# nghorbani/moshpp

Hardware: AMD Instinct MI355X
Metric: solved mocap frames/sec (Stage-II) (higher is better)
Workload: dtype f64

## Files before the change

### moshpp_amd/csrc/chain_solve.hip

```cpp
#include "moshii_dev.h"
#include <utility>
#include <type_traits>
#if defined(__HIP_DEVICE_COMPILE__)
#define MOSHII_OPAQUE(x) __asm__ __volatile__("" : "+v"(x))
#else
#define MOSHII_OPAQUE(x) do {} while (0)
#endif
__device__ __forceinline__ double uni64(double v) {
#if defined(__HIP_DEVICE_COMPILE__)
    return __hiloint2double(__builtin_amdgcn_readfirstlane(__double2hiint(v)), __builtin_amdgcn_readfirstlane(__double2loint(v)));
#else
    return v;
#endif
}

namespace moshii {

typedef double v2d __attribute__((vector_size(16)));

#ifdef MOSHII_PROFILE
__device__ long long g_prof[64];
#define MOSHII_TRACE_N 8192
__device__ long long g_trace[8][MOSHII_TRACE_N][4];
#define TRACE_STAMP(co, seq, ev) do { if (threadIdx.x == 0 && blockIdx.x < 8u * (co).G && (blockIdx.x & 7u) == 0u && (seq) < MOSHII_TRACE_N) g_trace[(co).rank][(seq)][(ev)] = wall_clock64(); } while (0)
#define PROF_BEGIN() long long _pt = clock64()
#define PROF_LAP(slot) do { __syncthreads(); if (threadIdx.x == 0 && blockIdx.x == 0) { long long _n = clock64(); g_prof[slot] += _n - _pt; _pt = _n; } else { _pt = 0; } } while (0)
#define PROF_COUNT(slot) do { if (threadIdx.x == 0 && blockIdx.x == 0) g_prof[slot] += 1; } while (0)
#define PROF_MARK() do { if (threadIdx.x == 0 && blockIdx.x == 0) g_prof[63] = clock64(); } while (0)
#define PROF_LAP_EXT(slot) do { __syncthreads(); if (threadIdx.x == 0 && blockIdx.x == 0) { long long _n = clock64(); g_prof[slot] += _n - g_prof[63]; g_prof[63] = _n; } } while (0)
#define PROF_T(var) const long long var = clock64()
#define PROF_ACC(slot, var) do { if (threadIdx.x == 0 && blockIdx.x == 0) g_prof[slot] += clock64() - var; } while (0)
#else
#define PROF_BEGIN() do {} while (0)
#define PROF_LAP(slot) do {} while (0)
#define PROF_COUNT(slot) do {} while (0)
#define PROF_MARK() do {} while (0)
#define PROF_LAP_EXT(slot) do {} while (0)
#define PROF_T(var) do {} while (0)
#define PROF_ACC(slot, var) do {} while (0)
#define TRACE_STAMP(co, seq, ev) do {} while (0)
#endif

enum { S_KBEST = 0, S_PRIOR_SS = 1, S_FAIL = 2, S_TMP0 = 3, S_TMP1 = 4, S_TMP2 = 5, S_TMP3 = 6, S_PRIOR_REF = 7, S_PRIOR_KB0 = 8, S_BATON = 9, S_ABORT = 10,
       S_V0 = 11, S_V1 = 12,
       S_COOP_SEQ = 13, S_COOP_FAIL = 14
     };

struct Ctx {
    double *pose, *trans, *pose_t, *trans_t, *pose_prev, *vtarget, *fullpose;
    double *feat, *B, *omega, *Rw, *tw, *Rloc, *acol, *Jl;
    double *vposed, *vpos, *msim, *res, *vconst, *vshp, *shp0;
    double *xb, *ell, *score, *px0, *ps0;
    double *g, *dsd, *dgn, *ddl, *y;
    double *red, *scal;
    unsigned long long* anc;
    int *visidx, *colpid, *colprior, *pid2prior, *jointslot, *kfree, *colq, *ksum, *kconst;
    double *big, *Jh, *Jrow, *Lm, *Trot, *xjs, *rest;
    int* tjs;
};

struct FrameParams {
    const double* obs;
    double wt_data, wt_pose, wt_poseH, wt_velo;
    int has_velo, use_fingers, nobs;
    double wt_poseF;
    int use_face, use_shape, has_stay;
    int v0, v1;
};

struct Sse { double data, prior, velo, hand, total, face, shape, stay; };

template <int CTRL>
__device__ __forceinline__ double dpp_f64(double v) {
    const int lo = __builtin_amdgcn_update_dpp(0, __double2loint(v), CTRL, 0xf, 0xf, false);
    const int hi = __builtin_amdgcn_update_dpp(0, __double2hiint(v), CTRL, 0xf, 0xf, false);
    return __hiloint2double(hi, lo);
}
__device__ __forceinline__ double readlane_f64(double v, int lane ) {
    const int lo = __builtin_amdgcn_readlane(__double2loint(v), lane);
    const int hi = __builtin_amdgcn_readlane(__double2hiint(v), lane);
    return __hiloint2double(hi, lo);
}
enum { DPP_QUAD_1032 = 0xB1, DPP_QUAD_2301 = 0x4E, DPP_ROW_HALF_MIRROR = 0x141, DPP_ROW_MIRROR = 0x140 };
#if defined(__HIP_DEVICE_COMPILE__)
template <int K> __device__ __forceinline__ double rowbcast_f64(double v) {
    double r;
    asm volatile("s_nop 1\n\tv_mov_b64_dpp %0, %1 row_newbcast:%2 row_mask:0xf bank_mask:0xf" : "=v"(r) : "v"(v), "n"(K));
    return r;
}
template <int K, bool SETTLE = false> __device__ __forceinline__ void fmac_rowbcast(double& acc, double m, double a) {
    if constexpr (SETTLE) asm volatile("s_nop 1\n\tv_fmac_f64_dpp %0, -%1, %2 row_newbcast:%3 row_mask:0xf bank_mask:0xf" : "+v"(acc) : "v"(m), "v"(a), "n"(K));
    else asm volatile("v_fmac_f64_dpp %0, -%1, %2 row_newbcast:%3 row_mask:0xf bank_mask:0xf" : "+v"(acc) : "v"(m), "v"(a), "n"(K));
}
#else
template <int K> __device__ __forceinline__ double rowbcast_f64(double v) { return __shfl(v, K, 16); }
template <int K, bool SETTLE = false> __device__ __forceinline__ void fmac_rowbcast(double& acc, double m, double a) { acc = fma(-__shfl(m, K, 16), a, acc); }
#endif

__device__ __forceinline__ double wave_sum(double v) {
    v += dpp_f64<DPP_QUAD_1032>(v);
    v += dpp_f64<DPP_QUAD_2301>(v);
    v += dpp_f64<DPP_ROW_HALF_MIRROR>(v);
    v += dpp_f64<DPP_ROW_MIRROR>(v);
    return (readlane_f64(v, 0) + readlane_f64(v, 16)) + (readlane_f64(v, 32) + readlane_f64(v, 48));
}
__device__ __forceinline__ void wave_sum3(double& a, double& b, double& c) {
    a += dpp_f64<DPP_QUAD_1032>(a); b += dpp_f64<DPP_QUAD_1032>(b); c += dpp_f64<DPP_QUAD_1032>(c);
    a += dpp_f64<DPP_QUAD_2301>(a); b += dpp_f64<DPP_QUAD_2301>(b); c += dpp_f64<DPP_QUAD_2301>(c);
    a += dpp_f64<DPP_ROW_HALF_MIRROR>(a); b += dpp_f64<DPP_ROW_HALF_MIRROR>(b); c += dpp_f64<DPP_ROW_HALF_MIRROR>(c);
    a += dpp_f64<DPP_ROW_MIRROR>(a); b += dpp_f64<DPP_ROW_MIRROR>(b); c += dpp_f64<DPP_ROW_MIRROR>(c);
    a = (readlane_f64(a, 0) + readlane_f64(a, 16)) + (readlane_f64(a, 32) + readlane_f64(a, 48));
    b = (readlane_f64(b, 0) + readlane_f64(b, 16)) + (readlane_f64(b, 32) + readlane_f64(b, 48));
    c = (readlane_f64(c, 0) + readlane_f64(c, 16)) + (readlane_f64(c, 32) + readlane_f64(c, 48));
}
__device__ __forceinline__ double wave_max(double v) {
    v = fmax(v, dpp_f64<DPP_QUAD_1032>(v));
    v = fmax(v, dpp_f64<DPP_QUAD_2301>(v));
    v = fmax(v, dpp_f64<DPP_ROW_HALF_MIRROR>(v));
    v = fmax(v, dpp_f64<DPP_ROW_MIRROR>(v));
    return fmax(fmax(readlane_f64(v, 0), readlane_f64(v, 16)), fmax(readlane_f64(v, 32), readlane_f64(v, 48)));
}

__device__ __forceinline__ void block_sum3(double& a, double& b, double& c, double* red) {
    wave_sum3(a, b, c);
    __syncthreads();
    const int tid = threadIdx.x;
    if ((tid & 63) == 0) { red[(tid >> 6) * 3 + 0] = a; red[(tid >> 6) * 3 + 1] = b; red[(tid >> 6) * 3 + 2] = c; }
    __syncthreads();
    a = (red[0] + red[3]) + (red[6] + red[9]);
    b = (red[1] + red[4]) + (red[7] + red[10]);
    c = (red[2] + red[5]) + (red[8] + red[11]);
}
__device__ __forceinline__ void block_sum4(double& a, double& b, double& c, double& d, double* red) {
    wave_sum3(a, b, c);
    d = wave_sum(d);
    __syncthreads();
    const int tid = threadIdx.x;
    if ((tid & 63) == 0) { red[(tid >> 6) * 4 + 0] = a; red[(tid >> 6) * 4 + 1] = b; red[(tid >> 6) * 4 + 2] = c; red[(tid >> 6) * 4 + 3] = d; }
    __syncthreads();
    a = (red[0] + red[4]) + (red[8] + red[12]);
    b = (red[1] + red[5]) + (red[9] + red[13]);
    c = (red[2] + red[6]) + (red[10] + red[14]);
    d = (red[3] + red[7]) + (red[11] + red[15]);
}
__device__ __forceinline__ void block_max_sum3(double& mx, double& a, double& b, double& c, double* red) {
    wave_sum3(a, b, c);
    mx = wave_max(mx);
    __syncthreads();
    const int tid = threadIdx.x;
    if ((tid & 63) == 0) { red[(tid >> 6) * 4 + 0] = a; red[(tid >> 6) * 4 + 1] = b; red[(tid >> 6) * 4 + 2] = c; red[(tid >> 6) * 4 + 3] = mx; }
    __syncthreads();
    a = (red[0] + red[4]) + (red[8] + red[12]);
    b = (red[1] + red[5]) + (red[9] + red[13]);
    c = (red[2] + red[6]) + (red[10] + red[14]);
    mx = fmax(fmax(red[3], red[7]), fmax(red[11], red[15]));
}
__device__ __forceinline__ double block_sum(double a, double* red) {
    double b = 0.0, c = 0.0;
    block_sum3(a, b, c, red);
    return a;
}
__device__ __forceinline__ double block_max(double a, double* red) {
    a = wave_max(a);
    __syncthreads();
    const int tid = threadIdx.x;
    if ((tid & 63) == 0) red[tid >> 6] = a;
    __syncthreads();
    return fmax(fmax(red[0], red[1]), fmax(red[2], red[3]));
}

#if defined(__HIP_DEVICE_COMPILE__)
#define MOSHII_DRAIN_VMEM() asm volatile("s_waitcnt vmcnt(0)" ::: "memory")
#else
#define MOSHII_DRAIN_VMEM() do {} while (0)
#endif
__device__ __forceinline__ unsigned long long f64_bits(double v) { unsigned long long b; __builtin_memcpy(&b, &v, 8); return b; }
__device__ __forceinline__ double bits_f64(unsigned long long b) { double v; __builtin_memcpy(&v, &b, 8); return v; }
__device__ __forceinline__ void coop_st(MOSHII_GP(unsigned long long) p, double v) {
    __hip_atomic_store(p, f64_bits(v), __ATOMIC_RELAXED, __HIP_MEMORY_SCOPE_AGENT);
}
__device__ __forceinline__ double coop_ld(MOSHII_GP(unsigned long long) p) {
    return bits_f64(__hip_atomic_load(p, __ATOMIC_RELAXED, __HIP_MEMORY_SCOPE_AGENT));
}
#if defined(__HIP_DEVICE_COMPILE__)
__device__ __forceinline__ void coop_st_l2(MOSHII_GP(unsigned long long) p, unsigned long long v) {
    asm volatile("global_store_dwordx2 %0, %1, off sc0" :: "v"(p), "v"(v) : "memory");
}
__device__ __forceinline__ unsigned long long coop_ld_l2(MOSHII_GP(unsigned long long) p) {
    unsigned long long v;
    asm volatile("global_load_dwordx2 %0, %1, off sc0 nt\n\ts_waitcnt vmcnt(0)" : "=v"(v) : "v"(p) : "memory");
    return v;
}
__device__ __forceinline__ void coop_st32_l2(MOSHII_GP(unsigned int) p, unsigned v) {
    asm volatile("global_store_dword %0, %1, off sc0" :: "v"(p), "v"(v) : "memory");
}
__device__ __forceinline__ unsigned coop_ld32_l2(MOSHII_GP(unsigned int) p) {
    unsigned v;
    asm volatile("global_load_dword %0, %1, off sc0 nt\n\ts_waitcnt vmcnt(0)" : "=v"(v) : "v"(p) : "memory");
    return v;
}
#endif
template <bool L2> __device__ __forceinline__ void coop_st64(MOSHII_GP(unsigned long long) p, unsigned long long v) {
#if defined(__HIP_DEVICE_COMPILE__)
    if constexpr (L2) { coop_st_l2(p, v); return; }
#endif
    __hip_atomic_store(p, v, __ATOMIC_RELAXED, __HIP_MEMORY_SCOPE_AGENT);
}
template <bool L2> __device__ __forceinline__ unsigned long long coop_ld64(MOSHII_GP(unsigned long long) p) {
#if defined(__HIP_DEVICE_COMPILE__)
    if constexpr (L2) return coop_ld_l2(p);
#endif
    return __hip_atomic_load(p, __ATOMIC_RELAXED, __HIP_MEMORY_SCOPE_AGENT);
}
template <bool L2> __device__ __forceinline__ void coop_st32(MOSHII_GP(unsigned int) p, unsigned v) {
#if defined(__HIP_DEVICE_COMPILE__)
    if constexpr (L2) { coop_st32_l2(p, v); return; }
#endif
    __hip_atomic_store(p, v, __ATOMIC_RELAXED, __HIP_MEMORY_SCOPE_AGENT);
}
template <bool L2> __device__ __forceinline__ unsigned coop_ld32(MOSHII_GP(unsigned int) p) {
#if defined(__HIP_DEVICE_COMPILE__)
    if constexpr (L2) return coop_ld32_l2(p);
#endif
    return __hip_atomic_load(p, __ATOMIC_RELAXED, __HIP_MEMORY_SCOPE_AGENT);
}
__device__ __forceinline__ unsigned coop_begin(const Ctx& cx) { return (unsigned)__builtin_amdgcn_readfirstlane((int)cx.scal[S_COOP_SEQ]) + 1u; }
__device__ __forceinline__ MOSHII_GP(unsigned long long) coop_slot(const CoopCtx& co, unsigned seq, int r) {
    return co.slots + ((size_t)(seq & 1u) * co.G + r) * co.slot_doubles;
}
#if defined(__HIP_DEVICE_COMPILE__) && !defined(MOSHII_COOP_NO_BUF)
typedef unsigned coop_u4 __attribute__((ext_vector_type(4)));
struct CoopSlot { __amdgpu_buffer_rsrc_t rs; };
__device__ __forceinline__ CoopSlot coop_slot16(const CoopCtx& co, unsigned seq, int r) {
    CoopSlot cs;
    cs.rs = __builtin_amdgcn_make_buffer_rsrc((void*)coop_slot(co, seq, r), 0, co.slot_doubles * 8, 0x00020000);
    return cs;
}
template <bool L2 = false>
__device__ __forceinline__ void coop_st16(const CoopSlot& cs, int off16, double a, double b) {
    const unsigned long long ba = f64_bits(a), bb = f64_bits(b);
    const coop_u4 v = {(unsigned)ba, (unsigned)(ba >> 32), (unsigned)bb, (unsigned)(bb >> 32)};
    if constexpr (L2) __builtin_amdgcn_raw_buffer_store_b128(v, cs.rs, off16 * 16, 0, 1);
    else __builtin_amdgcn_raw_buffer_store_b128(v, cs.rs, off16 * 16, 0, 16);
}
template <bool L2 = false>
__device__ __forceinline__ void coop_ld16(const CoopSlot& cs, int off16, double& a, double& b) {
    coop_u4 v;
    if constexpr (L2) v = __builtin_amdgcn_raw_buffer_load_b128(cs.rs, off16 * 16, 0, 3);
    else v = __builtin_amdgcn_raw_buffer_load_b128(cs.rs, off16 * 16, 0, 16);
    a = bits_f64(((unsigned long long)v[1] << 32) | v[0]);
    b = bits_f64(((unsigned long long)v[3] << 32) | v[2]);
}
#else
struct CoopSlot { MOSHII_GP(unsigned long long) p; };
__device__ __forceinline__ CoopSlot coop_slot16(const CoopCtx& co, unsigned seq, int r) { CoopSlot cs; cs.p = coop_slot(co, seq, r); return cs; }
template <bool L2 = false>
__device__ __forceinline__ void coop_st16(const CoopSlot& cs, int off16, double a, double b) { coop_st(cs.p + 2 * (size_t)off16, a); coop_st(cs.p + 2 * (size_t)off16 + 1, b); }
template <bool L2 = false>
__device__ __forceinline__ void coop_ld16(const CoopSlot& cs, int off16, double& a, double& b) { a = coop_ld(cs.p + 2 * (size_t)off16); b = coop_ld(cs.p + 2 * (size_t)off16 + 1); }
#endif
__device__ __forceinline__ void coop_skew(const CoopCtx& co, unsigned seq) {
    if (co.skew != 0) {
        unsigned h = (seq * 2654435761u) ^ ((unsigned)co.rank * 40503u + (unsigned)co.skew * 977u);
        h ^= h >> 13; h *= 0x5bd1e995u; h ^= h >> 15;
        for (unsigned i = h & 3u; i > 0u; --i) __builtin_amdgcn_s_sleep(127);
    }
}
template <bool L2 = false>
__device__ __forceinline__ bool coop_publish_wait(const CoopCtx& co, const Ctx& cx, unsigned seq) {
    const int tid = threadIdx.x;
    coop_skew(co, seq);
    PROF_T(_tp0);
    MOSHII_DRAIN_VMEM();
    __syncthreads();
    PROF_ACC(33, _tp0);
    PROF_T(_tp1);
#if defined(MOSHII_COOP_FENCES)
    if (tid == 0) __hip_atomic_store(co.flags + co.rank, seq, __ATOMIC_RELEASE, __HIP_MEMORY_SCOPE_AGENT);
#else
    if (tid == 0) coop_st32<L2>(co.flags + co.rank, seq);
#endif
    TRACE_STAMP(co, seq, 1);
    if (tid < co.G && cx.scal[S_COOP_FAIL] == 0.0) {
        bool ok = true;
        unsigned spins = 0;
        while ((int)(coop_ld32<L2>(co.flags + tid) - seq) < 0) {
            __builtin_amdgcn_s_sleep(1);
            if ((++spins & 255u) == 0u)
                if (spins > (1u << 21) || __hip_atomic_load(co.flags + co.G, __ATOMIC_RELAXED, __HIP_MEMORY_SCOPE_AGENT) != 0u) { ok = false; break; }
        }
        if (!ok) {
            __hip_atomic_store(co.flags + co.G, 1u, __ATOMIC_RELAXED, __HIP_MEMORY_SCOPE_AGENT);
            cx.scal[S_COOP_FAIL] = 1.0;
        }
    }
    __syncthreads();
#if defined(MOSHII_COOP_FENCES)
    __builtin_amdgcn_fence(__ATOMIC_ACQUIRE, "agent");
#endif
    PROF_ACC(34, _tp1);
    TRACE_STAMP(co, seq, 2);
    return cx.scal[S_COOP_FAIL] == 0.0;
}
__device__ __forceinline__ void coop_end(const Ctx& cx, unsigned seq) {
    __syncthreads();
    if (threadIdx.x == 0) cx.scal[S_COOP_SEQ] = (double)seq;
    __syncthreads();
}
template <int NS, bool L2>
__device__ __forceinline__ bool coop_exchange_small_(const CoopCtx& co, const Ctx& cx, unsigned seq, const double (&mine)[NS], double* land) {
    const int tid = threadIdx.x;
    const int goff = co.slot_doubles - 32;
    coop_skew(co, seq);
    if (tid < 2 * NS) {
        double v = mine[0];
#pragma unroll
        for (int k = 1; k < NS; ++k) if ((tid >> 1) == k) v = mine[k];
        const unsigned long long b = f64_bits(v);
        const unsigned half = (tid & 1) ? (unsigned)(b >> 32) : (unsigned)b;
        coop_st64<L2>(coop_slot(co, seq, co.rank) + goff + tid, ((unsigned long long)seq << 32) | half);
    }
    TRACE_STAMP(co, seq, 1);
    if (tid < co.G * 2 * NS && cx.scal[S_COOP_FAIL] == 0.0) {
        const int r = tid / (2 * NS), k = tid - r * 2 * NS;
        auto* g = coop_slot(co, seq, r) + goff + k;
        unsigned long long x;
        unsigned spins = 0;
        bool ok = true;
        while (((x = coop_ld64<L2>(g)) >> 32) != seq) {
            __builtin_amdgcn_s_sleep(1);
            if ((++spins & 255u) == 0u)
                if (spins > (1u << 21) || __hip_atomic_load(co.flags + co.G, __ATOMIC_RELAXED, __HIP_MEMORY_SCOPE_AGENT) != 0u) { ok = false; break; }
        }
        if (!ok) {
            __hip_atomic_store(co.flags + co.G, 1u, __ATOMIC_RELAXED, __HIP_MEMORY_SCOPE_AGENT);
            cx.scal[S_COOP_FAIL] = 1.0;
        }
        reinterpret_cast<unsigned*>(land)[tid] = (unsigned)x;
    }
    __syncthreads();
    TRACE_STAMP(co, seq, 2);
    return cx.scal[S_COOP_FAIL] == 0.0;
}
template <int NS>
__device__ __forceinline__ bool coop_exchange_small(const CoopCtx& co, const Ctx& cx, unsigned seq, const double (&mine)[NS], double* land) {
    return coop_exchange_small_<NS, false>(co, cx, seq, mine, land);
}

__device__ __forceinline__ void rodrigues_dev(const double* r, double* R, double* Jl) {
    const double x = r[0], y = r[1], z = r[2];
    const double t2 = x * x + y * y + z * z;
    double a, b, c;
    if (t2 < 1e-6) {
        a = 1.0 - t2 / 6.0 + t2 * t2 / 120.0;
        b = 0.5 - t2 / 24.0 + t2 * t2 / 720.0;
        c = 1.0 / 6.0 - t2 / 120.0 + t2 * t2 / 5040.0;
    } else {
        const double t = sqrt(t2);
        double s, co;
        sincos(t, &s, &co);
        a = s / t;
        b = (1.0 - co) / t2;
        c = (t - s) / (t2 * t);
    }
    const double K2[9] = {x * x - t2, x * y, x * z, x * y, y * y - t2, y * z, x * z, y * z, z * z - t2};
    const double Km[9] = {0.0, -z, y, z, 0.0, -x, -y, x, 0.0};
#pragma unroll
    for (int e = 0; e < 9; ++e) {
        const double id = (e == 0 || e == 4 || e == 8) ? 1.0 : 0.0;
        R[e] = id + a * Km[e] + b * K2[e];
        Jl[e] = id + b * Km[e] + c * K2[e];
    }
}

__device__ __forceinline__ void rodrigues_R(const double* r, double* R) {
    const double x = r[0], y = r[1], z = r[2];
    const double t2 = x * x + y * y + z * z;
    double a, b;
    if (t2 < 1e-6) {
        a = 1.0 - t2 / 6.0 + t2 * t2 / 120.0;
        b = 0.5 - t2 / 24.0 + t2 * t2 / 720.0;
    } else {
        const double t = sqrt(t2);
        double s, co;
        sincos(t, &s, &co);
        a = s / t;
        b = (1.0 - co) / t2;
    }
    const double K2[9] = {x * x - t2, x * y, x * z, x * y, y * y - t2, y * z, x * z, y * z, z * z - t2};
    const double Km[9] = {0.0, -z, y, z, 0.0, -x, -y, x, 0.0};
#pragma unroll
    for (int e = 0; e < 9; ++e) R[e] = ((e == 0 || e == 4 || e == 8) ? 1.0 : 0.0) + a * Km[e] + b * K2[e];
}

__device__ __forceinline__ void mat3_mul(const double* A, const double* Bm, double* C) {
#pragma unroll
    for (int i = 0; i < 3; ++i)
#pragma unroll
        for (int j = 0; j < 3; ++j)
            C[i * 3 + j] = A[i * 3 + 0] * Bm[0 * 3 + j] + A[i * 3 + 1] * Bm[1 * 3 + j] + A[i * 3 + 2] * Bm[2 * 3 + j];
}
__device__ __forceinline__ void mat3_vec(const double* A, double x, double y, double z, double& ox, double& oy, double& oz) {
    ox = A[0] * x + A[1] * y + A[2] * z;
    oy = A[3] * x + A[4] * y + A[5] * z;
    oz = A[6] * x + A[7] * y + A[8] * z;
}

__device__ __forceinline__ void marker_eval(const double* c, const double* v0, const double* v1, const double* v2,
                                            double* mk, double* L ) {
    const double e1[3] = {v1[0] - v0[0], v1[1] - v0[1], v1[2] - v0[2]};
    const double e2[3] = {v2[0] - v0[0], v2[1] - v0[1], v2[2] - v0[2]};
    const double l1 = sqrt(e1[0] * e1[0] + e1[1] * e1[1] + e1[2] * e1[2]);
    const double f1[3] = {e1[0] / l1, e1[1] / l1, e1[2] / l1};
    const double nv[3] = {e1[1] * e2[2] - e1[2] * e2[1], e1[2] * e2[0] - e1[0] * e2[2], e1[0] * e2[1] - e1[1] * e2[0]};
    const double ln = sqrt(nv[0] * nv[0] + nv[1] * nv[1] + nv[2] * nv[2]);
    const double f2[3] = {nv[0] / ln, nv[1] / ln, nv[2] / ln};
    const double f3[3] = {f1[1] * f2[2] - f1[2] * f2[1], f1[2] * f2[0] - f1[0] * f2[2], f1[0] * f2[1] - f1[1] * f2[0]};
#pragma unroll
    for (int i = 0; i < 3; ++i) mk[i] = v0[i] + c[0] * f1[i] + c[1] * f2[i] + c[2] * f3[i];
    if (L == nullptr) return;
    double D1[9], D2[9];
#pragma unroll
    for (int i = 0; i < 3; ++i)
#pragma unroll
        for (int j = 0; j < 3; ++j) {
            const double id = (i == j) ? 1.0 : 0.0;
            D1[i * 3 + j] = (id - f1[i] * f1[j]) / l1;
            D2[i * 3 + j] = (id - f2[i] * f2[j]) / ln;
        }
    const double N1[9] = {0.0, e2[2], -e2[1], -e2[2], 0.0, e2[0], e2[1], -e2[0], 0.0};
    const double N2[9] = {0.0, -e1[2], e1[1], e1[2], 0.0, -e1[0], -e1[1], e1[0], 0.0};
    double F21[9], F22[9];
    mat3_mul(D2, N1, F21);
    mat3_mul(D2, N2, F22);
    const double S1[9] = {0.0, -f1[2], f1[1], f1[2], 0.0, -f1[0], -f1[1], f1[0], 0.0};
    const double S2[9] = {0.0, -f2[2], f2[1], f2[2], 0.0, -f2[0], -f2[1], f2[0], 0.0};
    double T1[9], T2[9], T3[9];
    mat3_mul(S2, D1, T1);
    mat3_mul(S1, F21, T2);
    mat3_mul(S1, F22, T3);
#pragma unroll
    for (int i = 0; i < 3; ++i)
#pragma unroll
        for (int j = 0; j < 3; ++j) {
            const int e = i * 3 + j;
            const double de1 = c[0] * D1[e] + c[1] * F21[e] + c[2] * (T2[e] - T1[e]);
            const double de2 = c[1] * F22[e] + c[2] * T3[e];
            const double id = (i == j) ? 1.0 : 0.0;
            L[i * 9 + j] = id - de1 - de2;
            L[i * 9 + 3 + j] = de1;
            L[i * 9 + 6 + j] = de2;
        }
}

__device__ __forceinline__ double fullpose_entry(const ModelDev& md, const double* pose, int d) {
    const int bd = md.body_dof, nhf = md.nhand_full;
    if (d < bd) return pose[d];
    const int h = d - bd;
    const int lo = md.col_lo[h], hi = md.col_hi[h];
    double v0 = md.hands_mean[h], v1 = 0.0;
    int i = lo;
    for (; i + 2 <= hi; i += 2) {
        v0 += pose[bd + i] * md.comps[i * nhf + h];
        v1 += pose[bd + i + 1] * md.comps[(i + 1) * nhf + h];
    }
    if (i < hi) v0 += pose[bd + i] * md.comps[i * nhf + h];
    return v0 + v1;
}

__device__ __forceinline__ void posedirs_partial(const Ctx& cx, const AttachDev& at, const int* klist, int nk,
                                                 const double* base, double* dst) {
    const int tid = threadIdx.x;
    const int Nv = at.Nv, Nvp = at.Nvp, Nvh = Nvp >> 1;
    for (int it = tid; it < 3 * Nvh; it += MOSHII_TPB) {
        const int i = it / Nvh, a2 = it - i * Nvh;
        double s0x = 0.0, s0y = 0.0, s1x = 0.0, s1y = 0.0, s2x = 0.0, s2y = 0.0;
        const auto* pp = gptr(reinterpret_cast<const v2d*>(at.Pt)) + (size_t)(i * 9) * Nvh + a2;
        constexpr int PB = 3;
        for (int idx0 = 0; idx0 < nk; idx0 += PB) {
            v2d q[PB][9];
            int kk[PB];
#pragma unroll
            for (int u = 0; u < PB; ++u) {
                kk[u] = klist[min(idx0 + u, nk - 1)];
                const auto* pk = pp + (size_t)((kk[u] - 1) * 27) * Nvh;
#pragma unroll
                for (int e = 0; e < 9; ++e) q[u][e] = pk[(size_t)e * Nvh];
            }
#pragma unroll
            for (int u = 0; u < PB; ++u) {
                if (idx0 + u < nk) {
                    const double* f = &cx.feat[kk[u] * 9];
#pragma unroll
                    for (int e = 0; e < 9; e += 3) {
                        s0x += q[u][e][0] * f[e]; s0y += q[u][e][1] * f[e];
                        s1x += q[u][e + 1][0] * f[e + 1]; s1y += q[u][e + 1][1] * f[e + 1];
                        s2x += q[u][e + 2][0] * f[e + 2]; s2y += q[u][e + 2][1] * f[e + 2];
                    }
// ... 1616 lines not shown
                                    for (int i = 0; i < 4; ++i) acc.c[t][i] += own[4 * t + i];
                                }
                        } else if (wanted(r0 + u)) {
#pragma unroll
                            for (int t = 0; t < NT; ++t)
                                if (4 * t + wv < NE) {
#pragma unroll
                                    for (int i = 0; i < 4; ++i) acc.c[t][i] += v[u][4 * t + i];
                                }
                        }
                    }
                }
                if (has_prior) {
                    if (NUP + RB * NUA > 48) {
#pragma unroll
                        for (int u = 0; u < NUP; ++u) coop_ld16<L2>(sp, (NUA + u) * MOSHII_TPB + tid, pv[2 * u], pv[2 * u + 1]);
                    }
#pragma unroll
                    for (int e = 0; e < NE; ++e) pblk[e] = pv[e];
                    gqp = pv[NE];
                }
                }
            }
        };
        exchange(std::false_type());
        if (tid < n) cx.dgn[tid] = gqp;
        TRACE_STAMP(co, seq, 3);
        coop_end(cx, seq);
        PROF_LAP(32);
    }
    A.take(acc, cx.big);
    {
        const int ty = tid >> 4, tx = tid & 15, bn = n >> 4;
        if (ty == (n & 15)) {
#pragma unroll
            for (int bi = 0; bi < NBLK; ++bi)
#pragma unroll
                for (int bj = 0; bj <= bi; ++bj)
                    if (bi == bn && bj * 16 + tx < n) cx.g[bj * 16 + tx] = -A.a[bi * (bi + 1) / 2 + bj];
        }
        __syncthreads();
    }
    double* dvec = cx.y;
    const int kb = (np_ > 0) ? (int)cx.scal[S_KBEST] : 0;
    for (int q = tid; q < n; q += MOSHII_TPB) {
        double dg = 0.0, gq = 0.0;
        if (XT && q >= ncp) {
            const int e = q - ncp;
            const double sv_ = pose[md.NP + e];
            const double w2 = op.wt_shape * op.wt_shape;
            dg += w2; gq -= w2 * sv_;
            if (fp.has_stay) { const double y2 = op.wt_shape_stay * op.wt_shape_stay; dg += y2; gq -= y2 * (sv_ - cx.shp0[e]); }
        } else if (q >= 3) {
            const int pid = cx.colpid[q];
            if (fp.has_velo) { const double w2 = fp.wt_velo * fp.wt_velo; dg += w2; gq -= w2 * (pose[pid] - cx.vtarget[pid]); }
            const int pb = cx.colprior[q];
            if (COOP) { gq += cx.dgn[q]; }
            else if (pb >= 0) {
                const auto* Hk = pr.halfprec + (size_t)kb * np_ * np_ + pb;
                const auto* mu = pr.means + (size_t)kb * np_;
                double s0 = 0.0, s1 = 0.0;
                for (int b0 = 0; b0 < np_; b0 += 32) {
                    double h[32];
#pragma unroll
                    for (int k = 0; k < 32; ++k) h[k] = Hk[(size_t)min(b0 + k, np_ - 1) * np_];
#pragma unroll
                    for (int k = 0; k < 32; k += 2) {
                        const int b = b0 + k;
                        s0 = fma(h[k] * ((b < np_) ? 1.0 : 0.0), cx.xb[min(b, np_ - 1)] - mu[min(b, np_ - 1)], s0);
                        s1 = fma(h[k + 1] * ((b + 1 < np_) ? 1.0 : 0.0), cx.xb[min(b + 1, np_ - 1)] - mu[min(b + 1, np_ - 1)], s1);
                    }
                }
                gq -= fp.wt_pose * fp.wt_pose * (s0 + s1);
            }
            if (fp.use_fingers) {
                if (op.nfinger > 0 && pid >= op.finger[0] && pid <= op.finger[op.nfinger - 1]) {
                    const double w2 = fp.wt_poseH * fp.wt_poseH; dg += w2; gq -= w2 * pose[pid];
                }
            }
            if constexpr (XT) {
                if (fp.use_face && op.nface > 0 && pid >= op.face[0] && pid <= op.face[op.nface - 1]) {
                    const double w2 = fp.wt_poseF * fp.wt_poseF; dg += w2; gq -= w2 * pose[pid];
                }
            }
            if (op.njangle > 0)
                for (int i = 0; i < op.njangle; ++i)
                    if (op.jangle[i] == pid) {
                        const double e = exp(pose[pid]);
                        const double r = (e * e) * (fp.wt_pose * op.wt_jangle), d = 2.0 * r;
                        dg += d * d; gq -= d * r;
                    }
        }
        dvec[q] = dg;
        cx.g[q] += gq;
    }
    __syncthreads();
    A.add_diag(dvec, n);
    if constexpr (COOP) {
#pragma unroll
        for (int e = 0; e < AReg<NBLK>::NE; ++e) A.a[e] += pblk[e];
    } else {
        if (np_ > 0) A.add_prior(fp.wt_pose * fp.wt_pose, pr.halfprec + (size_t)kb * np_ * np_, np_, cx.colprior, n);
    }
    __syncthreads();
    PROF_LAP(8);
}

__device__ __forceinline__ Ctx make_ctx(double* lds, const ChainLayout& ly) {
    Ctx cx;
    cx.pose = lds + ly.o_pose; cx.trans = lds + ly.o_trans; cx.pose_t = lds + ly.o_pose_t; cx.trans_t = lds + ly.o_trans_t;
    cx.pose_prev = lds + ly.o_pose_prev; cx.vtarget = lds + ly.o_vtarget; cx.fullpose = lds + ly.o_fullpose;
    cx.Jl = lds + ly.o_Jl; cx.feat = lds + ly.o_feat; cx.B = lds + ly.o_B; cx.omega = lds + ly.o_omega; cx.Rw = lds + ly.o_Rw; cx.tw = lds + ly.o_tw;
    cx.Rloc = lds + ly.o_Rloc; cx.acol = lds + ly.o_acol;
    cx.vshp = lds + ly.o_vshp; cx.shp0 = lds + ly.o_shp0;
    cx.vconst = lds + ly.o_vconst; cx.vposed = lds + ly.o_vposed; cx.vpos = lds + ly.o_vpos; cx.msim = lds + ly.o_msim; cx.res = lds + ly.o_res;
    cx.xb = lds + ly.o_xb; cx.ell = lds + ly.o_ell; cx.score = lds + ly.o_score; cx.px0 = lds + ly.o_px0; cx.ps0 = lds + ly.o_ps0;
    cx.g = lds + ly.o_g; cx.dsd = lds + ly.o_dsd; cx.dgn = lds + ly.o_dgn; cx.ddl = lds + ly.o_ddl; cx.y = lds + ly.o_y;
    cx.red = lds + ly.o_red; cx.scal = lds + ly.o_scal;
    cx.anc = reinterpret_cast<unsigned long long*>(lds + ly.o_anc);
    int* ints = reinterpret_cast<int*>(lds + ly.o_ints);
    cx.visidx = ints + ly.i_visidx; cx.colpid = ints + ly.i_colpid; cx.colprior = ints + ly.i_colprior;
    cx.pid2prior = ints + ly.i_pid2prior; cx.jointslot = ints + ly.i_jointslot; cx.kfree = ints + ly.i_kfree;
    cx.colq = ints + ly.i_colq; cx.ksum = ints + ly.i_ksum; cx.kconst = ints + ly.i_kconst;
    cx.big = lds + ly.o_big;
    cx.Jh = cx.big + ly.t_Jh; cx.Jrow = cx.big + ly.t_Jrow; cx.Lm = cx.big + ly.t_Lm; cx.Trot = cx.big + ly.t_Trot;
    cx.xjs = cx.big + ly.t_xjs; cx.rest = cx.big + ly.t_rest;
    cx.tjs = reinterpret_cast<int*>(cx.big + ly.t_tjs);

    return cx;
}

template <class T>
__device__ __forceinline__ T uniform_load(const T* p) {
    static_assert(sizeof(T) % 4 == 0, "word-sized descriptors only");
    T out;
    int* o = reinterpret_cast<int*>(&out);
    const int* q = reinterpret_cast<const int*>(p);
#pragma unroll
    for (int i = 0; i < (int)(sizeof(T) / 4); ++i) o[i] = __builtin_amdgcn_readfirstlane(q[i]);
    return out;
}

struct KArgsMirror { const ChainDev* chains; ModelDev md; PriorDev pr; OptsDev op; ChainLayout ly; int n_chains; };
#if defined(__HIP_DEVICE_COMPILE__) && !defined(MOSHII_NO_KARGS)
typedef const KArgsMirror __attribute__((address_space(4)))* KArgsPtr;
__device__ __forceinline__ KArgsPtr kargs_of(const KernelCtx* kc) {
    const unsigned long long v = kc->kargs;
    return (KArgsPtr)(((unsigned long long)(unsigned)__builtin_amdgcn_readfirstlane((int)(v >> 32)) << 32) | (unsigned)__builtin_amdgcn_readfirstlane((int)v));
}
#define MOSHII_CTX_FROM_KARGS(kc) const KArgsPtr ka_ = kargs_of(kc); const ChainLayout ly = ka_->ly; const ModelDev md = ka_->md; const PriorDev pr = ka_->pr; const OptsDev op = ka_->op;
#else
#define MOSHII_CTX_FROM_KARGS(kc) const ChainLayout ly = uniform_load(&(kc)->ly); const ModelDev md = uniform_load(&(kc)->md); const PriorDev pr = uniform_load(&(kc)->pr); const OptsDev op = uniform_load(&(kc)->op);
#endif

template <int NBLK>
__device__ __noinline__ bool coop_rs_reduce(unsigned seq_) {
    extern __shared__ __attribute__((aligned(16))) double lds[];
    const KernelCtx* kc = reinterpret_cast<const KernelCtx*>(lds);
    const ChainLayout ly = uniform_load(&kc->ly);
    const Ctx cx = make_ctx(lds, ly);
    const CoopCtx co = uniform_load(&kc->co);
    constexpr int NT = JtJAcc<NBLK>::NT, NE = AReg<NBLK>::NE;
    const int tid = threadIdx.x;
    const int wv = __builtin_amdgcn_readfirstlane(tid >> 6);
    unsigned seq = (unsigned)__builtin_amdgcn_readfirstlane((int)seq_);
    const int TPR = (NT + co.G - 1) / co.G, tlo = co.rank * TPR, thi = min(NT, tlo + TPR);
    v4d sums[NT];
#pragma unroll
    for (int t = 0; t < NT; ++t)
        if (t >= tlo && t < thi && 4 * t + wv < NE) {
            double v[MOSHII_COOP_MAXG][4];
#pragma unroll
            for (int r = 0; r < MOSHII_COOP_MAXG; ++r)
                if (r < co.G) {
                    const CoopSlot sr = coop_slot16(co, seq, r);
                    coop_ld16(sr, (2 * t) * MOSHII_TPB + tid, v[r][0], v[r][1]);
                    coop_ld16(sr, (2 * t + 1) * MOSHII_TPB + tid, v[r][2], v[r][3]);
                }
            v4d sum = v4d{0.0, 0.0, 0.0, 0.0};
#pragma unroll
            for (int r = 0; r < MOSHII_COOP_MAXG; ++r)
                if (r < co.G) {
#pragma unroll
                    for (int i = 0; i < 4; ++i) sum[i] += v[r][i];
                }
            sums[t] = sum;
        }
    coop_end(cx, seq);
    seq = coop_begin(cx);
    const CoopSlot mine2 = coop_slot16(co, seq, co.rank);
#pragma unroll
    for (int t = 0; t < NT; ++t)
        if (t >= tlo && t < thi && 4 * t + wv < NE) {
            coop_st16(mine2, (2 * t) * MOSHII_TPB + tid, sums[t][0], sums[t][1]);
            coop_st16(mine2, (2 * t + 1) * MOSHII_TPB + tid, sums[t][2], sums[t][3]);
        }
    return coop_publish_wait(co, cx, seq);
}

template <bool XT, bool COOP>
__device__ __noinline__ Sse eval_forward_fn(const uint8_t* visrow, int o_pose, int o_trans, int i_klist, int nk,
                                            int o_vbase, int light) {
    extern __shared__ __attribute__((aligned(16))) double lds[];
    const KernelCtx* kc = reinterpret_cast<const KernelCtx*>(lds);
    MOSHII_CTX_FROM_KARGS(kc)
    const AttachDev at = uniform_load(&kc->at);
    const FrameParams fp = uniform_load(reinterpret_cast<const FrameParams*>(kc->fp_raw));
    const Ctx cx = make_ctx(lds, ly);
    const int* ints = reinterpret_cast<const int*>(lds + ly.o_ints);
    CoopCtx co = CoopCtx();
    if constexpr (COOP) co = uniform_load(&kc->co);
    return eval_forward<XT, COOP>(cx, md, at, pr, op, lds + __builtin_amdgcn_readfirstlane(o_pose), lds + __builtin_amdgcn_readfirstlane(o_trans),
                                  fp, visrow, ints + __builtin_amdgcn_readfirstlane(i_klist), __builtin_amdgcn_readfirstlane(nk),
                                  lds + __builtin_amdgcn_readfirstlane(o_vbase), __builtin_amdgcn_readfirstlane(light) != 0, co);
}

#ifdef MOSHII_ASM_INLINE
#define MOSHII_ASM_LINKAGE __forceinline__
#else
#define MOSHII_ASM_LINKAGE __noinline__
#endif
template <int NBLK, bool XT, bool COOP>
__device__ MOSHII_ASM_LINKAGE typename APass<NBLK, MOSHII_ASM_RET_VEC(NBLK)>::type assemble_fn(int o_pose, int n, int ncp, int nkf, int nfree_hand, double* qs) {
    extern __shared__ __attribute__((aligned(16))) double lds[];
    const KernelCtx* kc = reinterpret_cast<const KernelCtx*>(lds);
    MOSHII_CTX_FROM_KARGS(kc)
    const AttachDev at = uniform_load(&kc->at);
    const FrameParams fp = uniform_load(reinterpret_cast<const FrameParams*>(kc->fp_raw));
    const Ctx cx = make_ctx(lds, ly);
    AReg<NBLK> A;
    CoopCtx co = CoopCtx();
    if constexpr (COOP) co = uniform_load(&kc->co);
    assemble<NBLK, XT, COOP>(cx, ly, md, at, pr, op, lds + __builtin_amdgcn_readfirstlane(o_pose), fp, __builtin_amdgcn_readfirstlane(n),
                             __builtin_amdgcn_readfirstlane(ncp), __builtin_amdgcn_readfirstlane(nkf), __builtin_amdgcn_readfirstlane(nfree_hand), qs, A, co);
    return APass<NBLK, MOSHII_ASM_RET_VEC(NBLK)>::pack(A);
}

__device__ __noinline__ void rigid_init_serial(const Ctx& cx, const FrameParams& fp, const uint8_t* visrow, int M) {
    double am[3] = {0, 0, 0}, bm[3] = {0, 0, 0};
    int cnt = 0;
    for (int m = 0; m < M; ++m) if (visrow[m]) {
        for (int i = 0; i < 3; ++i) { am[i] += cx.msim[m * 3 + i]; bm[i] += fp.obs[m * 3 + i]; }
        ++cnt;
    }
    for (int i = 0; i < 3; ++i) { am[i] /= cnt; bm[i] /= cnt; }
    double G[9] = {0, 0, 0, 0, 0, 0, 0, 0, 0};
    for (int m = 0; m < M; ++m) if (visrow[m])
        for (int i = 0; i < 3; ++i) for (int j = 0; j < 3; ++j)
            G[i * 3 + j] += (cx.msim[m * 3 + i] - am[i]) * (fp.obs[m * 3 + j] - bm[j]);
    double V[9] = {1, 0, 0, 0, 1, 0, 0, 0, 1};
    for (int sweep = 0; sweep < 60; ++sweep) {
        double off = 0.0;
        for (int p = 0; p < 2; ++p) for (int q = p + 1; q < 3; ++q) {
            double al = 0, be = 0, ga = 0;
            for (int i = 0; i < 3; ++i) { al += G[i * 3 + p] * G[i * 3 + p]; be += G[i * 3 + q] * G[i * 3 + q]; ga += G[i * 3 + p] * G[i * 3 + q]; }
            if (fabs(ga) <= 1e-300 || fabs(ga) <= 1e-17 * sqrt(al * be)) continue;
            off = fmax(off, fabs(ga) / sqrt(al * be));
            const double zeta = (be - al) / (2.0 * ga);
            const double t = ((zeta >= 0) ? 1.0 : -1.0) / (fabs(zeta) + sqrt(1.0 + zeta * zeta));
            const double c = 1.0 / sqrt(1.0 + t * t), s = c * t;
            for (int i = 0; i < 3; ++i) {
                const double gp = G[i * 3 + p], gq = G[i * 3 + q];
                G[i * 3 + p] = c * gp - s * gq; G[i * 3 + q] = s * gp + c * gq;
                const double vp = V[i * 3 + p], vq = V[i * 3 + q];
                V[i * 3 + p] = c * vp - s * vq; V[i * 3 + q] = s * vp + c * vq;
            }
        }
        if (off < 1e-15) break;
    }
    double sv[3], U[9];
    int imin = 0, imax = 0;
    for (int c = 0; c < 3; ++c) {
        sv[c] = sqrt(G[0 * 3 + c] * G[0 * 3 + c] + G[1 * 3 + c] * G[1 * 3 + c] + G[2 * 3 + c] * G[2 * 3 + c]);
        if (sv[c] < sv[imin]) imin = c;
        if (sv[c] > sv[imax]) imax = c;
    }
    for (int c = 0; c < 3; ++c) for (int i = 0; i < 3; ++i) U[i * 3 + c] = (sv[c] > 0) ? G[i * 3 + c] / sv[c] : 0.0;
    if (sv[imin] <= 1e-13 * sv[imax]) {
        const int c1 = (imin + 1) % 3, c2 = (imin + 2) % 3;
        U[0 * 3 + imin] = U[1 * 3 + c1] * U[2 * 3 + c2] - U[2 * 3 + c1] * U[1 * 3 + c2];
        U[1 * 3 + imin] = U[2 * 3 + c1] * U[0 * 3 + c2] - U[0 * 3 + c1] * U[2 * 3 + c2];
        U[2 * 3 + imin] = U[0 * 3 + c1] * U[1 * 3 + c2] - U[1 * 3 + c1] * U[0 * 3 + c2];
    }
    double R[9];
    for (int i = 0; i < 3; ++i) for (int j = 0; j < 3; ++j)
        R[i * 3 + j] = V[i * 3 + 0] * U[j * 3 + 0] + V[i * 3 + 1] * U[j * 3 + 1] + V[i * 3 + 2] * U[j * 3 + 2];
    const double det = R[0] * (R[4] * R[8] - R[5] * R[7]) - R[1] * (R[3] * R[8] - R[5] * R[6]) + R[2] * (R[3] * R[7] - R[4] * R[6]);
    if (det < 0.0)
        for (int i = 0; i < 3; ++i) for (int j = 0; j < 3; ++j) R[i * 3 + j] -= 2.0 * V[i * 3 + imin] * U[j * 3 + imin];
    double rx = R[7] - R[5], ry = R[2] - R[6], rz = R[3] - R[1];
    const double s = sqrt((rx * rx + ry * ry + rz * rz) * 0.25);
    double c = (R[0] + R[4] + R[8] - 1.0) * 0.5;
    c = fmin(1.0, fmax(-1.0, c));
    const double theta = acos(c);
    double rv[3];
    if (s < 1e-5) {
        if (c > 0) { rv[0] = rv[1] = rv[2] = 0.0; }
        else {
            double x = sqrt(fmax((R[0] + 1.0) * 0.5, 0.0));
            double y = sqrt(fmax((R[4] + 1.0) * 0.5, 0.0)) * ((R[1] >= 0) ? 1.0 : -1.0);
            double z = sqrt(fmax((R[8] + 1.0) * 0.5, 0.0)) * ((R[2] >= 0) ? 1.0 : -1.0);
            if (fabs(x) < fabs(y) && fabs(x) < fabs(z) && ((R[5] > 0) != (y * z > 0))) z = -z;
            const double nn = sqrt(x * x + y * y + z * z);
            rv[0] = x * theta / nn; rv[1] = y * theta / nn; rv[2] = z * theta / nn;
        }
    } else {
        const double k = 0.5 * theta / s;
        rv[0] = rx * k; rv[1] = ry * k; rv[2] = rz * k;
    }
    cx.pose[0] = rv[0]; cx.pose[1] = rv[1]; cx.pose[2] = rv[2];
    for (int i = 0; i < 3; ++i) cx.trans[i] = bm[i] - (R[i * 3 + 0] * am[0] + R[i * 3 + 1] * am[1] + R[i * 3 + 2] * am[2]);
}

template <int NBLK, bool XT, bool COOP>
__device__ Sse run_phase(const Ctx& cx, const ChainLayout& ly, const ModelDev& md, const AttachDev& at, const PriorDev& pr,
                         const OptsDev& op, const FrameParams& fp, const uint8_t* visrow, MOSHII_GP(const int) ids, int nids, int nshp,
                         double* qs, double e3,
                         bool rigid, bool eval_only, bool reuse, Sse& carried, bool& at_pose, int& fwd_set, int set_id, int& vc_key,
                         int& tab_key, int& n_iter, int& n_fev, int& fail, const CoopCtx& co) {
    const int tid = threadIdx.x;
    const int ncp = 3 + nids;
    const int n = ncp + (XT ? nshp : 0);
    const int NPX = XT ? ly.NPX : md.NP;
    if (!eval_only && tab_key != set_id) {
        tab_key = set_id;
        for (int i = tid; i < md.NP; i += MOSHII_TPB) cx.colq[i] = -1;
        __syncthreads();
        for (int q = tid; q < n; q += MOSHII_TPB) {
            const int pid = (q < 3) ? -1 : ((q < ncp) ? ids[q - 3] : md.NP + (q - ncp));
            cx.colpid[q] = pid;
            cx.colprior[q] = (pid >= 0 && pid < md.NP) ? cx.pid2prior[pid] : -1;
            if (pid >= 0 && pid < md.NP) cx.colq[pid] = q;
        }
        if (tid == 0) {
            for (int k = 0; k < md.K; ++k) cx.jointslot[k] = -1;
            for (int i = 0; i < nids; ++i) {
                const int pid = ids[i];
                if (pid < md.body_dof) cx.jointslot[pid / 3] = 0;
                else for (int k = md.body_dof / 3; k < md.K; ++k) cx.jointslot[k] = 0;
            }
            int c = 0;
            for (int k = 0; k < md.K; ++k) if (cx.jointslot[k] == 0) { cx.jointslot[k] = c; cx.kfree[c] = k; ++c; }
            cx.scal[S_TMP0] = (double)c;
            int nh = 0;
            for (int i = 0; i < nids; ++i) nh += (ids[i] >= md.body_dof) ? 1 : 0;
            cx.scal[S_TMP2] = (double)nh;
            int ns = 0, nc = 0;
            for (int k = 1; k < md.K; ++k) { if (cx.jointslot[k] >= 0) cx.ksum[ns++] = k; else cx.kconst[nc++] = k; }
            cx.scal[S_TMP3] = (double)ns;
        }
        __syncthreads();
    }
    const int nkf = (int)cx.scal[S_TMP0], nfree_hand = (int)cx.scal[S_TMP2];
    const int nks = (int)cx.scal[S_TMP3];
    const int nkc = md.K - 1 - nks;
    if (vc_key != set_id) {
        for (int d = tid; d < md.P; d += MOSHII_TPB) cx.fullpose[d] = fullpose_entry(md, cx.pose, d);
        __syncthreads();
        if (tid < md.K) {
            double R[9];
            rodrigues_R(&cx.fullpose[3 * tid], R);
#pragma unroll
            for (int e = 0; e < 9; ++e) cx.feat[tid * 9 + e] = R[e] - ((e == 0 || e == 4 || e == 8) ? 1.0 : 0.0);
        }
        __syncthreads();
        if constexpr (COOP) posedirs_partial_range(cx, at, cx.kconst, nkc, at.vsh, cx.vconst, 3 * co.mlo, 3 * co.mhi);
        else posedirs_partial(cx, at, cx.kconst, nkc, at.vsh, cx.vconst);
        __syncthreads();
        vc_key = set_id;
    }
    AReg<NBLK> A;
    A.zero();
    if (tid == 0) {
        extern __shared__ __attribute__((aligned(16))) double lds[];
        static_assert(sizeof(FrameParams) <= sizeof(KernelCtx::fp_raw), "KernelCtx::fp_raw too small");
        *reinterpret_cast<FrameParams*>(reinterpret_cast<KernelCtx*>(lds)->fp_raw) = fp;
    }
    for (int i = tid; i < NPX; i += MOSHII_TPB) cx.pose_t[i] = cx.pose[i];
    if (tid < 3) cx.trans_t[tid] = cx.trans[tid];
    __syncthreads();
    Sse last;
    double sse = 0.0, delta = op.delta0, norm_sd = 0.0, norm_gn = 0.0, step = 0.0, p2 = 0.0, gd = 0.0;
    double dAd = 0.0, dl_dd = 0.0, dl_gs = 0.0, dl_ds = 0.0;
    bool init = true, done = false, have_gn = false;
    int iteration = 0;
    bool skip_eval = reuse && !rigid;
    int light = (!rigid && at_pose && fwd_set == set_id) ? 1 : 0;
    while (true) {
        int tid = threadIdx.x; MOSHII_OPAQUE(tid);
        if (skip_eval) { last = carried; skip_eval = false; }
        else { PROF_T(_te); last = eval_forward_fn<XT, COOP>(visrow, ly.o_pose_t, ly.o_trans_t, ly.i_ksum, nks, ly.o_vconst, light); PROF_ACC(15, _te); }
        if constexpr (COOP) { if (cx.scal[S_COOP_FAIL] != 0.0) break; }
        if (!(last.total == last.total)) { fail = 1; break; }
        light = 0;
        at_pose = true;
        fwd_set = set_id;
        if (rigid) {
            if constexpr (COOP) {
                const unsigned seq = coop_begin(cx);
                auto gather = [&](auto l2) {
                    constexpr bool L2 = decltype(l2)::value;
                    auto* mine = coop_slot(co, seq, co.rank);
                    for (int i = 3 * co.mlo + tid; i < 3 * co.mhi; i += MOSHII_TPB) coop_st64<L2>(mine + i, f64_bits(cx.msim[i]));
                    if (tid == 0) coop_st64<L2>(mine + 3 * at.M, f64_bits((double)co.mlo));
                    if (coop_publish_wait<L2>(co, cx, seq)) {
                        const int M3 = 3 * at.M;
                        for (int i = tid; i < M3; i += MOSHII_TPB) {
                            int r = 0;
                            for (int q = 1; q < co.G; ++q) r += (i >= 3 * (int)bits_f64(coop_ld64<L2>(coop_slot(co, seq, q) + 3 * at.M))) ? 1 : 0;
                            if (r != co.rank) cx.msim[i] = bits_f64(coop_ld64<L2>(coop_slot(co, seq, r) + i));
                        }
                    }
                };
                gather(std::false_type());
                coop_end(cx, seq);
            }
            if (tid == 0) rigid_init_serial(cx, fp, visrow, at.M);
            __syncthreads();
            for (int i = tid; i < NPX; i += MOSHII_TPB) cx.pose_t[i] = cx.pose[i];
            if (tid < 3) cx.trans_t[tid] = cx.trans[tid];
            __syncthreads();
            rigid = false;
            continue;
        }
        if (eval_only) break;
        ++n_fev;
        PROF_T(_t1);
        bool improved = false, do_assemble = false;
        double rho = 0.0;
        if (init) {
            sse = uni64(last.total);
            do_assemble = true;
        } else {
            rho = sse - last.total;
            if (rho > 0.0) rho = rho / (2.0 * gd - dAd);
            improved = rho > 0.0;
            at_pose = improved;
            if (improved) {
                for (int i = tid; i < NPX; i += MOSHII_TPB) cx.pose[i] = cx.pose_t[i];
                if (tid < 3) cx.trans[tid] = cx.trans_t[tid];
                __syncthreads();
                if (e3 > 0.0 && (sse - last.total) / sse < e3) done = true;
                else { do_assemble = true; sse = uni64(last.total); }
            }
        }
        PROF_ACC(23, _t1);
        double pp = 0.0, gg = 0.0, gAg = 0.0;
        if (do_assemble) {
            { PROF_T(_ta); A = APass<NBLK, MOSHII_ASM_RET_VEC(NBLK)>::unpack(assemble_fn<NBLK, XT, COOP>(ly.o_pose, n, ncp, nkf, nfree_hand, qs)); PROF_ACC(16, _ta); }
            if constexpr (COOP) { if (cx.scal[S_COOP_FAIL] != 0.0) break; }
            PROF_T(_t2);
            double gm = 0.0;
            for (int q = tid; q < n; q += MOSHII_TPB) {
                const double gq = cx.g[q];
                const double pq = (q < 3) ? cx.trans[q] : cx.pose[cx.colpid[q]];
                gm = fmax(gm, fabs(gq)); pp += pq * pq; gg += gq * gq;
            }
            gAg = A.quad_partial(cx.g, n, tid);
            block_max_sum3(gm, pp, gg, gAg, cx.red);
            gm = uni64(gm); pp = uni64(pp); gg = uni64(gg); gAg = uni64(gAg);
            if (gm < 1e-15) done = true;
            PROF_ACC(24, _t2);
        }
        PROF_T(_t3);
        if (!init) {
            const double pnorm2 = (improved && do_assemble) ? pp : p2;
            if (rho > 0.9) delta = fmax(delta, 2.5 * step);
            else if (rho < 0.05) delta *= 0.25;
            delta = uni64(delta);
            if (delta <= 1e-15 * sqrt(pnorm2)) done = true;
        }
        if (init || improved) {
            if (!init && iteration >= op.maxiter) done = true;
            if (done) break;
            ++iteration;
            const double csd = gg / gAg;
            norm_sd = uni64(fabs(csd) * sqrt(gg));
            for (int q = tid; q < n; q += MOSHII_TPB) cx.dsd[q] = csd * cx.g[q];
            have_gn = false;
            __syncthreads();
        } else if (done) {
            break;
        }
        init = false;
        PROF_ACC(25, _t3);
        PROF_T(_t4);
        if (norm_sd >= delta) {
            const double sc = delta / norm_sd;
            for (int q = tid; q < n; q += MOSHII_TPB) cx.ddl[q] = sc * cx.dsd[q];
        } else {
            if (!have_gn) {
                constexpr bool BIG = XT && NBLK > 8;
                bool solved;
                PROF_T(_ts);
                if constexpr (BIG) solved = ldl_big<NBLK>(A, qs + (size_t)6 * md.K * op.nshape, cx.big, cx.g, cx.dgn, cx.y, n);
                else solved = ldl_solve<NBLK>(A, ly.o_big, ly.o_g, ly.o_dgn, ly.o_y, n);
                PROF_ACC(17, _ts);
                PROF_ACC(26, _t4);
                if (!solved) {
                    fail = 1;
                    for (int q = tid; q < n; q += MOSHII_TPB) cx.dgn[q] = cx.dsd[q];
                    __syncthreads();
                }
                double sg = 0.0;
                dl_dd = 0.0; dl_gs = 0.0; dl_ds = 0.0;
                for (int q = tid; q < n; q += MOSHII_TPB) {
                    const double dg_ = cx.dgn[q], dsq = cx.dsd[q], df = dg_ - dsq;
                    sg += dg_ * dg_; dl_dd += df * df; dl_gs += dg_ * dsq; dl_ds += df * dsq;
                }
                block_sum4(sg, dl_dd, dl_gs, dl_ds, cx.red);
                dl_dd = uni64(dl_dd); dl_gs = uni64(dl_gs); dl_ds = uni64(dl_ds);
                norm_gn = uni64(sqrt(sg));
                have_gn = true;
            }
            if (norm_gn <= delta) {
                for (int q = tid; q < n; q += MOSHII_TPB) cx.ddl[q] = cx.dgn[q];
            } else {
                const double delta_sq = delta * delta;
                const double sqnorm_sd = norm_sd * norm_sd;
                const double pnow = dl_dd * delta_sq + dl_gs * dl_gs - (norm_gn * norm_gn) * sqnorm_sd;
                const double beta = (delta_sq - sqnorm_sd) / (dl_ds + sqrt(pnow));
                for (int q = tid; q < n; q += MOSHII_TPB) cx.ddl[q] = cx.dsd[q] + beta * (cx.dgn[q] - cx.dsd[q]);
            }
        }
        __syncthreads();
        PROF_T(_t5);
        double s2 = 0.0;
        p2 = 0.0; gd = 0.0;
        for (int q = tid; q < n; q += MOSHII_TPB) {
            const double dq = cx.ddl[q];
            const double pq = (q < 3) ? cx.trans[q] : cx.pose[cx.colpid[q]];
            s2 += dq * dq; p2 += pq * pq; gd += cx.g[q] * dq;
        }
        dAd = A.quad_partial(cx.ddl, n, tid);
        block_sum4(s2, p2, gd, dAd, cx.red);
        p2 = uni64(p2); gd = uni64(gd); dAd = uni64(dAd);
        step = uni64(sqrt(s2));
        if (step <= 1e-15 * sqrt(p2)) break;
        for (int i = tid; i < NPX; i += MOSHII_TPB) cx.pose_t[i] = cx.pose[i];
        if (tid < 3) cx.trans_t[tid] = cx.trans[tid] + cx.ddl[tid];
        __syncthreads();
        for (int q = 3 + tid; q < n; q += MOSHII_TPB) cx.pose_t[cx.colpid[q]] += cx.ddl[q];
        __syncthreads();
        PROF_ACC(27, _t5);
    }
    n_iter += iteration;
    carried = last;
    return last;
}


template <int NBLK, int MINW, bool XT, bool COOP = false>
__global__ __launch_bounds__(MOSHII_TPB, MINW) void k_chain_solve(const ChainDev* __restrict__ chains, ModelDev md, PriorDev pr,
                                                             OptsDev op, ChainLayout ly, int n_chains) {
    extern __shared__ __attribute__((aligned(16))) double lds[];
    const int tid = threadIdx.x;
    int chain_id = blockIdx.x;
    CoopCtx co = CoopCtx();
    if constexpr (COOP) {
        const int G = chains[0].coop.G;
        const int q = blockIdx.x >> 3;
        chain_id = 8 * (q / G) + (blockIdx.x & 7);
        if (chain_id >= n_chains) return;
        const ChainDev* c0 = chains + chain_id;
        co.G = G; co.rank = q % G; co.prior_rank = c0->coop.prior_rank;
        co.mlo = c0->coop.mlo[co.rank]; co.mhi = c0->coop.mlo[co.rank + 1];
        co.prior_bare = c0->coop.mlo[co.prior_rank + 1] == c0->coop.mlo[co.prior_rank];
        co.slot_doubles = c0->coop.slot_doubles; co.slots = c0->coop.slots; co.flags = c0->coop.flags; co.skew = c0->coop.skew;
    }
    const bool lead = !COOP || co.rank == 0;
    const ChainDev* chp = chains + chain_id;
    const AttachDev at = *chp->att;
    const Ctx cx = make_ctx(lds, ly);
    if (tid == 0) {
        KernelCtx* kc = reinterpret_cast<KernelCtx*>(lds);
        kc->ly = ly; kc->md = md; kc->pr = pr; kc->op = op; kc->at = at;
#if defined(__HIP_DEVICE_COMPILE__)
        kc->kargs = (unsigned long long)__builtin_amdgcn_kernarg_segment_ptr();
#if !defined(MOSHII_NO_KARGS)
        {
            const KArgsPtr kk = (KArgsPtr)__builtin_amdgcn_kernarg_segment_ptr();
            if (kk->chains != chains || kk->n_chains != n_chains || kk->ly.total_doubles != ly.total_doubles || kk->md.V != md.V || kk->op.maxiter != op.maxiter)
                __builtin_trap();
        }
#endif
#endif
        if constexpr (COOP) { kc->co = co; cx.scal[S_COOP_SEQ] = 0.0; cx.scal[S_COOP_FAIL] = 0.0; }
    }

    const int NP = md.NP, M = at.M, F = chp->F, skip = chp->skip;
    bool has_prev, first;
    {
        const double* is = chp->init_state;
        const double* ip = chp->init_pose;
        const double* iv = chp->init_prev;
        const double* it = chp->init_trans;
        for (int i = tid; i < NP; i += MOSHII_TPB) {
            cx.pose[i] = is ? is[i] : (ip ? ip[i] : 0.0);
            cx.pose_prev[i] = is ? is[NP + i] : (iv ? iv[i] : 0.0);
            cx.vtarget[i] = 0.0;
            cx.pid2prior[i] = -1;
        }
        if (tid < 3) cx.trans[tid] = is ? is[2 * NP + tid] : (it ? it[tid] : 0.0);
        if constexpr (XT) {
            const double* ish = chp->init_shape;
            for (int e = tid; e < op.nshape; e += MOSHII_TPB) { cx.pose[NP + e] = is ? is[2 * NP + 5 + e] : (ish ? ish[e] : 0.0); cx.shp0[e] = 0.0; }
        }
        has_prev = is ? (is[2 * NP + 3] != 0.0) : (iv != nullptr);
        first = is ? (is[2 * NP + 4] != 0.0) : (chp->first != 0);
    }
    if (tid == 0) cx.scal[S_PRIOR_REF] = 0.0;
    for (int i = tid; i < 8 * pr.npose + 16; i += MOSHII_TPB) cx.ell[i] = 0.0;
    if (tid < md.K) cx.anc[tid] = md.anc[tid];
    for (int i = tid; i < 3 * md.K; i += MOSHII_TPB) cx.Jl[i] = md.J[i];
    __syncthreads();
    for (int b = tid; b < op.nbody; b += MOSHII_TPB) cx.pid2prior[op.body[b]] = b;
    __syncthreads();
    int vc_key = 0, tab_key = 0;
    int rejoin_run = 0;
    int bi_next = 0;
    bool fuse_on = false;
    bool at_pose = false;
    int fwd_set = 0;
    PROF_BEGIN();
#ifdef MOSHII_PROFILE
    const long long _wall0 = wall_clock64();
#endif

    bool tail_cut = false;
    for (int t = 0; t <= F; ++t) {
        PROF_T(_tf);
        if constexpr (!COOP && !XT) {
            if (chp->tail_done != nullptr && chp->tail_can_cut != 0 && t < F && F - t > chp->tail_left) {
                if (tid == 0) cx.scal[S_ABORT] = (double)__hip_atomic_load(chp->tail_done, __ATOMIC_RELAXED, __HIP_MEMORY_SCOPE_AGENT);
                __syncthreads();
                const bool cut = cx.scal[S_ABORT] >= (double)chp->tail_quota;
                __syncthreads();
                if (cut) {
                    auto spoil = [&](double* so, double flag) {
                        for (int i = tid; i < NP; i += MOSHII_TPB) { so[i] = cx.pose[i]; so[NP + i] = cx.pose_prev[i]; }
                        if (tid < 3) so[2 * NP + tid] = cx.trans[tid];
                        if (tid == 3) so[2 * NP + 3] = flag;
                        if (tid == 4) so[2 * NP + 4] = 0.0;
                    };
                    spoil(chp->entry_state, MOSHII_MARK_ENTRY_SPOILED);
                    spoil(chp->final_state, MOSHII_MARK_FINAL_SPOILED);
                    if (tid == 0 && chp->tail_mark != nullptr) *chp->tail_mark = 0x7fffffff;
                    tail_cut = true;
                    break;
                }
            }
        }
        if constexpr (COOP) {
            if (chp->baton != nullptr || chp->nb > 0 || chp->rejoin_tol > 0.0) {
                bool halt = false;
                if (lead) {
                    const int S = 2 * NP + 5;
                    if (rejoin_run >= 2 && t < F) {
                        if (tid == 0 && chp->frames_done) *chp->frames_done = t;
                        halt = true;
                    }
                    if (!halt && bi_next < chp->nb && t == chp->bnd[bi_next] - chp->bnd_off) {
                        double* s1 = chp->run_final + (size_t)bi_next * S;
                        for (int i = tid; i < NP; i += MOSHII_TPB) { s1[i] = cx.pose[i]; s1[NP + i] = cx.pose_prev[i]; }
                        if (tid < 3) s1[2 * NP + tid] = cx.trans[tid];
                        if (tid == 3) s1[2 * NP + 3] = has_prev ? 1.0 : 0.0;
                        if (tid == 4) s1[2 * NP + 4] = first ? 1.0 : 0.0;
                        if (chp->baton != nullptr) {
                            if (tid == 0) {
                                int* st = chp->baton + 2 * (chp->chunk0 + 1 + bi_next);
                                double go = 1.0;
                                if (__hip_atomic_load(st, __ATOMIC_ACQUIRE, __HIP_MEMORY_SCOPE_AGENT) == 1) {
                                    __hip_atomic_store(st + 1, 1, __ATOMIC_RELEASE, __HIP_MEMORY_SCOPE_AGENT);
                                    int spins = 0;
                                    while (__hip_atomic_load(st, __ATOMIC_ACQUIRE, __HIP_MEMORY_SCOPE_AGENT) != 2) {
                                        __builtin_amdgcn_s_sleep(64);
                                        if (++spins > 20000) { go = 0.0; break; }
                                    }
                                }
                                __builtin_amdgcn_fence(__ATOMIC_ACQUIRE, "agent");
                                cx.scal[S_BATON] = go;
                            }
                            __syncthreads();
                            if (cx.scal[S_BATON] == 0.0) { if (tid == 0 && chp->frames_done) *chp->frames_done = t; halt = true; }
                            __syncthreads();
                        }
                        if (!halt) {
                            double* s2 = chp->run_entry + (size_t)(bi_next + 1) * S;
                            for (int i = tid; i < NP; i += MOSHII_TPB) { s2[i] = cx.pose[i]; s2[NP + i] = cx.pose_prev[i]; }
                            if (tid < 3) s2[2 * NP + tid] = cx.trans[tid];
                            if (tid == 3) s2[2 * NP + 3] = has_prev ? 1.0 : 0.0;
                            if (tid == 4) s2[2 * NP + 4] = first ? 1.0 : 0.0;
                            ++bi_next;
                        }
                    }
                    if (!halt && chp->baton != nullptr && t < F) {
                        if (tid == 0) cx.scal[S_ABORT] = (double)__hip_atomic_load(&chp->baton[2 * chp->chunk0 + 1], __ATOMIC_RELAXED, __HIP_MEMORY_SCOPE_AGENT);
                        __syncthreads();
                        if (cx.scal[S_ABORT] != 0.0) {
                            if (tid == 0) {
                                chp->run_entry[(size_t)bi_next * S + 2 * NP + 3] = MOSHII_MARK_ENTRY_SPOILED;
                                int* mark = chp->abort_at + chp->chunk0 + bi_next;
                                if (*mark < chp->bnd_off + t) *mark = chp->bnd_off + t;
                                if (chp->frames_done) *chp->frames_done = -t - 1;
                            }
                            halt = true;
                        }
                        __syncthreads();
                    }
                }
                const unsigned seq = coop_begin(cx);
                const double mine[1] = {halt ? 1.0 : 0.0};
                const bool okx = coop_exchange_small<1>(co, cx, seq, mine, cx.y);
                const double verdict = okx ? cx.y[0] : 1.0;
                coop_end(cx, seq);
                if (verdict != 0.0) break;
            }
        }
        for (int which = 0; which < 2; ++which) {
            double* so = (which == 0) ? ((t == skip) ? chp->entry_state : nullptr) : ((t == F) ? chp->final_state : nullptr);
            if (so == nullptr || !lead) continue;
            for (int i = tid; i < NP; i += MOSHII_TPB) { so[i] = cx.pose[i]; so[NP + i] = cx.pose_prev[i]; }
            if (tid < 3) so[2 * NP + tid] = cx.trans[tid];
            if (tid == 3) so[2 * NP + 3] = has_prev ? 1.0 : 0.0;
            if (tid == 4) so[2 * NP + 4] = first ? 1.0 : 0.0;
            if constexpr (XT) for (int e = tid; e < op.nshape; e += MOSHII_TPB) so[2 * NP + 5 + e] = cx.pose[NP + e];
        }
        if (!COOP && chp->fuse_flags != nullptr) {
            const int S = 2 * NP + 5 + (XT ? op.nshape : 0);
            if (t == skip && chp->entry_state != nullptr) {
                __syncthreads();
                if (tid == 0) { __threadfence(); __hip_atomic_store(&chp->fuse_flags[3 * chp->fuse_c], 1, __ATOMIC_RELEASE, __HIP_MEMORY_SCOPE_AGENT); }
            }
            if (chp->fuse_F == 0 && t == F) {
                __syncthreads();
                if (tid == 0) {
                    __threadfence();
                    __hip_atomic_store(&chp->fuse_flags[3 * chp->fuse_c + 1], 1, __ATOMIC_RELEASE, __HIP_MEMORY_SCOPE_AGENT);
                    __hip_atomic_store(&chp->fuse_flags[3 * chp->fuse_c + 2], 1, __ATOMIC_RELEASE, __HIP_MEMORY_SCOPE_AGENT);
                }
            }
            if (chp->fuse_F > 0 && t == chp->fuse_F) {
                double* sf = chp->run_final - S;
                for (int i = tid; i < NP; i += MOSHII_TPB) { sf[i] = cx.pose[i]; sf[NP + i] = cx.pose_prev[i]; }
                if (tid < 3) sf[2 * NP + tid] = cx.trans[tid];
                if (tid == 3) sf[2 * NP + 3] = has_prev ? 1.0 : 0.0;
                if (tid == 4) sf[2 * NP + 4] = first ? 1.0 : 0.0;
                if constexpr (XT) for (int e = tid; e < op.nshape; e += MOSHII_TPB) sf[2 * NP + 5 + e] = cx.pose[NP + e];
                __syncthreads();
                if (tid == 0) { __threadfence(); __hip_atomic_store(&chp->fuse_flags[3 * chp->fuse_c + 1], 1, __ATOMIC_RELEASE, __HIP_MEMORY_SCOPE_AGENT); }
                bool carry = false;
                auto state_dev = [&](const double* en) {
                    double dv = 0.0, nn = 0.0;
                    for (int i = tid; i < NP; i += MOSHII_TPB) { dv = fmax(dv, fmax(fabs(cx.pose[i] - en[i]), fabs(cx.pose_prev[i] - en[NP + i]))); nn += en[i] + en[NP + i]; }
                    if (tid < 3) dv = fmax(dv, fabs(cx.trans[tid] - en[2 * NP + tid]));
                    if (tid == 3 && (has_prev ? 1.0 : 0.0) != en[2 * NP + 3]) dv = MOSHII_HANDOFF_MISMATCH;
                    if (tid == 4 && (first ? 1.0 : 0.0) != en[2 * NP + 4]) dv = MOSHII_HANDOFF_MISMATCH;
                    if constexpr (XT) for (int e = tid; e < op.nshape; e += MOSHII_TPB) dv = fmax(dv, fabs(cx.pose[NP + e] - en[2 * NP + 5 + e]));
                    if (!(nn == nn)) dv = MOSHII_HANDOFF_MISMATCH;
                    return block_max(dv, cx.red);
                };
                auto wait_flag = [&](int* fl, int patience) {
                    if (tid == 0) {
                        double go = 1.0;
                        int spins = 0;
                        while (__hip_atomic_load(fl, __ATOMIC_ACQUIRE, __HIP_MEMORY_SCOPE_AGENT) != 1) {
                            __builtin_amdgcn_s_sleep(64);
                            if (++spins > patience) { go = 0.0; break; }
                        }
                        __builtin_amdgcn_fence(__ATOMIC_ACQUIRE, "agent");
                        cx.scal[S_BATON] = go;
                    }
                    __syncthreads();
                    const bool ok_ = cx.scal[S_BATON] != 0.0;
                    __syncthreads();
                    return ok_;
                };
                if (chp->fuse_has_next && wait_flag(chp->fuse_flags + 3 * (chp->fuse_c + 1), 2000)) {
                    const double dv = state_dev(chp->run_entry);
                    carry = !(dv <= chp->fuse_tol);
                    if (carry && dv > 1e-6 && chp->fuse_has_prev && wait_flag(chp->fuse_flags + 3 * (chp->fuse_c - 1) + 1, 150)) {
                        const double* lf = chp->run_final - 2 * S;
                        const double* oe = chp->run_entry - S;
                        double dl = 0.0;
                        for (int i = tid; i < 2 * NP + 3; i += MOSHII_TPB) dl = fmax(dl, fabs(lf[i] - oe[i]));
                        dl = block_max(dl, cx.red);
                        if (!(dl <= 1e-6)) carry = false;
                    }
                }
                if (carry && tid == 0) __hip_atomic_store(&chp->baton[2 * chp->chunk0], 1, __ATOMIC_RELEASE, __HIP_MEMORY_SCOPE_AGENT);
                __syncthreads();
                if (tid == 0) { __threadfence(); __hip_atomic_store(&chp->fuse_flags[3 * chp->fuse_c + 2], 1, __ATOMIC_RELEASE, __HIP_MEMORY_SCOPE_AGENT); }
                if (!carry) { if (tid == 0 && chp->frames_done) *chp->frames_done = t; break; }
                if (tid == 0) {
                    int* fl = chp->fuse_flags + 3 * (chp->fuse_c + 1) + 1;
                    double go = 1.0;
                    int spins = 0;
                    while (__hip_atomic_load(fl, __ATOMIC_ACQUIRE, __HIP_MEMORY_SCOPE_AGENT) != 1 ||
                           __hip_atomic_load(fl + 1, __ATOMIC_ACQUIRE, __HIP_MEMORY_SCOPE_AGENT) != 1) {
                        if (__hip_atomic_load(&chp->baton[2 * chp->chunk0 + 1], __ATOMIC_RELAXED, __HIP_MEMORY_SCOPE_AGENT) != 0) { go = 0.0; break; }
                        __builtin_amdgcn_s_sleep(64);
                        if (++spins > 20000) { go = 0.0; break; }
                    }
                    __builtin_amdgcn_fence(__ATOMIC_ACQUIRE, "agent");
                    if (go != 0.0 && chp->fuse_count != nullptr) atomicAdd(chp->fuse_count, 1);
                    cx.scal[S_BATON] = go;
                }
                __syncthreads();
                if (cx.scal[S_BATON] == 0.0) { if (tid == 0 && chp->frames_done) *chp->frames_done = t; break; }
                double* s2 = chp->run_entry;
                for (int i = tid; i < NP; i += MOSHII_TPB) { s2[i] = cx.pose[i]; s2[NP + i] = cx.pose_prev[i]; }
                if (tid < 3) s2[2 * NP + tid] = cx.trans[tid];
                if (tid == 3) s2[2 * NP + 3] = has_prev ? 1.0 : 0.0;
                if (tid == 4) s2[2 * NP + 4] = first ? 1.0 : 0.0;
                if constexpr (XT) for (int e = tid; e < op.nshape; e += MOSHII_TPB) s2[2 * NP + 5 + e] = cx.pose[NP + e];
                fuse_on = true;
            }
        }
        const bool sweeping = chp->fuse_F == 0 || fuse_on;
        if (!COOP && bi_next < chp->nb && t == chp->bnd[bi_next] - chp->bnd_off) {
            const int S = 2 * NP + 5 + (XT ? op.nshape : 0);
            double* s1 = chp->run_final + (size_t)bi_next * S;
            for (int i = tid; i < NP; i += MOSHII_TPB) { s1[i] = cx.pose[i]; s1[NP + i] = cx.pose_prev[i]; }
            if (tid < 3) s1[2 * NP + tid] = cx.trans[tid];
            if (tid == 3) s1[2 * NP + 3] = has_prev ? 1.0 : 0.0;
            if (tid == 4) s1[2 * NP + 4] = first ? 1.0 : 0.0;
            if constexpr (XT) for (int e = tid; e < op.nshape; e += MOSHII_TPB) s1[2 * NP + 5 + e] = cx.pose[NP + e];
            if (chp->baton != nullptr) {
                if (tid == 0) {
                    int* st = chp->baton + 2 * (chp->chunk0 + 1 + bi_next);
                    double go = 1.0;
                    if (chp->fuse_flags != nullptr) {
                        int* vd = chp->fuse_flags + 3 * (chp->chunk0 + bi_next) + 2;
                        int spins = 0;
                        while (__hip_atomic_load(vd, __ATOMIC_ACQUIRE, __HIP_MEMORY_SCOPE_AGENT) != 1) {
                            __builtin_amdgcn_s_sleep(64);
                            if (++spins > 20000) { go = 0.0; break; }
                        }
                    }
                    if (go != 0.0 && __hip_atomic_load(st, __ATOMIC_ACQUIRE, __HIP_MEMORY_SCOPE_AGENT) == 1) {
                        __hip_atomic_store(st + 1, 1, __ATOMIC_RELEASE, __HIP_MEMORY_SCOPE_AGENT);
                        int spins = 0;
                        while (__hip_atomic_load(st, __ATOMIC_ACQUIRE, __HIP_MEMORY_SCOPE_AGENT) != 2) {
                            __builtin_amdgcn_s_sleep(64);
                            if (++spins > 20000) { go = 0.0; break; }
                        }
                    }
                    if (go != 0.0 && chp->fuse_flags != nullptr) {
                        int* od = chp->fuse_flags + 3 * (chp->chunk0 + 1 + bi_next) + 1;
                        int spins = 0;
                        while (__hip_atomic_load(od, __ATOMIC_ACQUIRE, __HIP_MEMORY_SCOPE_AGENT) != 1) {
                            __builtin_amdgcn_s_sleep(64);
                            if (++spins > 20000) { go = 0.0; break; }
                        }
                    }
                    __builtin_amdgcn_fence(__ATOMIC_ACQUIRE, "agent");
                    cx.scal[S_BATON] = go;
                }
                __syncthreads();
                if (cx.scal[S_BATON] == 0.0) { if (tid == 0 && chp->frames_done) *chp->frames_done = t; break; }
            }
            double* s2 = chp->run_entry + (size_t)(bi_next + 1) * S;
            for (int i = tid; i < NP; i += MOSHII_TPB) { s2[i] = cx.pose[i]; s2[NP + i] = cx.pose_prev[i]; }
            if (tid < 3) s2[2 * NP + tid] = cx.trans[tid];
            if (tid == 3) s2[2 * NP + 3] = has_prev ? 1.0 : 0.0;
            if (tid == 4) s2[2 * NP + 4] = first ? 1.0 : 0.0;
            if constexpr (XT) for (int e = tid; e < op.nshape; e += MOSHII_TPB) s2[2 * NP + 5 + e] = cx.pose[NP + e];
            ++bi_next;
        }
        if (!COOP && chp->baton != nullptr && sweeping && t < F) {
            if (tid == 0) cx.scal[S_ABORT] = (double)__hip_atomic_load(&chp->baton[2 * chp->chunk0 + 1], __ATOMIC_RELAXED, __HIP_MEMORY_SCOPE_AGENT);
            __syncthreads();
            if (cx.scal[S_ABORT] != 0.0) {
                if (tid == 0) {
                    const int S = 2 * NP + 5 + (XT ? op.nshape : 0);
                    chp->run_entry[(size_t)bi_next * S + 2 * NP + 3] = MOSHII_MARK_ENTRY_SPOILED;
                    int* mark = chp->abort_at + chp->chunk0 + bi_next;
                    if (*mark < chp->bnd_off + t) *mark = chp->bnd_off + t;
                    if (chp->frames_done) *chp->frames_done = -t - 1;
                }
                break;
            }
        }
        if (t == F) break;
        const bool record = t >= skip;
        const uint8_t* visrow = chp->vis + (size_t)t * M;
        if (tid < 64) {
            int c = 0, c0 = 0, c1 = 0;
            for (int m0 = 0; m0 < M; m0 += 64) {
                const int m = m0 + tid;
                const bool v = m < M && gptr(visrow)[min(m, M - 1)] != 0;
                const unsigned long long mask = __ballot(v);
                if (v) cx.visidx[c + __popcll(mask & ((1ull << tid) - 1ull))] = m;
                c += __popcll(mask);
                if constexpr (COOP) {
                    c0 += __popcll(__ballot(v && m < co.mlo));
                    c1 += __popcll(__ballot(v && m < co.mhi));
                }
            }
            if (tid == 0) { cx.scal[S_TMP1] = (double)c; cx.scal[S_V0] = (double)c0; cx.scal[S_V1] = (double)c1; }
        }
        __syncthreads();
        const int nobs = (int)cx.scal[S_TMP1];
        if (nobs == 0) {
            int* st = chp->status;
            if (tid == 0 && st && record && lead) st[t] = 1;
            __syncthreads();
            continue;
        }
        FrameParams fp;
        fp.obs = chp->obs + (size_t)t * M * 3;
        fp.nobs = nobs;
        fp.v0 = COOP ? (int)cx.scal[S_V0] : 0;
        fp.v1 = COOP ? (int)cx.scal[S_V1] : nobs;
        const double n_miss = (double)(M - nobs);
        double anneal = 1.0;
        if (n_miss > 0.0) anneal = anneal + (n_miss / (double)M) * op.wt_annealing;
        fp.wt_data = op.wt_data * (op.num_train_markers / (double)nobs);
        const double wt_pose = op.wt_poseB * anneal;
        fp.wt_pose = wt_pose;
        fp.wt_poseH = op.wt_poseH * anneal;
        fp.wt_velo = op.wt_velo;
        fp.use_fingers = 0;
        fp.wt_poseF = 0.0; fp.use_face = 0; fp.use_shape = 0; fp.has_stay = 0;
        if constexpr (XT) {
            fp.wt_poseF = op.wt_poseF * anneal;
            fp.has_stay = (!first && op.wt_shape_stay != 0.0) ? 1 : 0;
            for (int e = tid; e < op.nshape; e += MOSHII_TPB) cx.shp0[e] = cx.pose[NP + e];
        }
        fp.has_velo = has_prev ? 1 : 0;
        if (has_prev)
            for (int i = tid; i < NP; i += MOSHII_TPB) cx.vtarget[i] = cx.pose[i] + (cx.pose[i] - cx.pose_prev[i]);
        if (!first) {
            for (int i = tid; i < NP; i += MOSHII_TPB) cx.pose_prev[i] = cx.pose[i];
            has_prev = true;
        }
        __syncthreads();
        int n_iter = 0, n_fev = 0, fail = 0;
        PROF_ACC(18, _tf);
        Sse fin, carried;
        const bool same_sets = op.same_sets != 0;
        double prev_wt_pose = -1.0;
        int prev_terms = -1;
        for (int kind = first ? 0 : 3; kind < 6; ++kind) {
            const bool round = kind < 3;
            const bool step2 = kind == 4;
            fp.wt_pose = round ? ((kind == 0) ? 10.0 : (kind == 1) ? 5.0 : 1.0) * wt_pose : wt_pose;
            fp.use_fingers = (kind >= 4 && op.nfinger > 0) ? 1 : 0;
            if constexpr (XT) {
                fp.use_face = (kind >= 4 && op.nface > 0) ? 1 : 0;
                fp.use_shape = (kind >= 4 && op.nshape > 0) ? 1 : 0;
            }
            const int terms = fp.use_fingers | (fp.use_face << 1) | (fp.use_shape << 2);
            const bool reuse = at_pose && prev_wt_pose == fp.wt_pose && prev_terms == terms;
            fin = run_phase<NBLK, XT, COOP>(cx, ly, md, at, pr, op, fp, visrow, step2 ? op.step2 : op.step1, step2 ? op.n2 : op.n1,
                                  (XT && step2) ? op.nshape : 0, XT ? chp->qscratch + (COOP ? (size_t)co.rank * chp->coop.qstride : 0) : nullptr,
                                  round ? op.e3_first : op.e3, kind == 0, kind == 5, reuse, carried, at_pose, fwd_set,
                                  (kind >= 4 && !same_sets) ? 2 : 1, vc_key, tab_key, n_iter, n_fev, fail, co);
            prev_wt_pose = fp.wt_pose; prev_terms = terms;
            if constexpr (COOP) { if (cx.scal[S_COOP_FAIL] != 0.0) break; }
        }
        if constexpr (COOP) {
            if (cx.scal[S_COOP_FAIL] != 0.0) break;
        }
        first = false;
        PROF_T(_tr);
        if (lead && record && sweeping && chp->rejoin_tol > 0.0 && chp->pose != nullptr && chp->trans != nullptr) {
            double dv = 0.0;
            const double* po = chp->pose + (size_t)t * NP;
            for (int i = tid; i < NP; i += MOSHII_TPB) dv = fmax(dv, fabs(cx.pose[i] - po[i]));
            if (tid < 3) dv = fmax(dv, fabs(cx.trans[tid] - chp->trans[t * 3 + tid]));
            if constexpr (XT)
                if (chp->shape != nullptr)
                    for (int e = tid; e < op.nshape; e += MOSHII_TPB) dv = fmax(dv, fabs(cx.pose[NP + e] - chp->shape[(size_t)t * op.nshape + e]));
            dv = block_max(dv, cx.red);
            rejoin_run = (dv <= chp->rejoin_tol) ? rejoin_run + 1 : 0;
        }
        if (record) {
            double* o;
            if (lead && (o = chp->pose) != nullptr) for (int i = tid; i < NP; i += MOSHII_TPB) o[(size_t)t * NP + i] = cx.pose[i];
            if (lead && (o = chp->fullpose) != nullptr) for (int i = tid; i < md.P; i += MOSHII_TPB) o[(size_t)t * md.P + i] = cx.fullpose[i];
            if ((o = chp->msim) != nullptr) {
                const int i_lo = COOP ? 3 * co.mlo : 0, i_hi = COOP ? 3 * co.mhi : 3 * M;
                for (int i = i_lo + tid; i < i_hi; i += MOSHII_TPB) o[(size_t)t * 3 * M + i] = cx.msim[i];
            }
            if constexpr (XT)
                if (lead && (o = chp->shape) != nullptr) for (int e = tid; e < op.nshape; e += MOSHII_TPB) o[(size_t)t * op.nshape + e] = cx.pose[NP + e];
            if (tid == 0 && lead) {
                if ((o = chp->trans) != nullptr) { o[t * 3 + 0] = cx.trans[0]; o[t * 3 + 1] = cx.trans[1]; o[t * 3 + 2] = cx.trans[2]; }
                if ((o = chp->errs) != nullptr) {
                    const bool ja = op.njangle > 0;
                    o[t * 8 + 0] = fin.data; o[t * 8 + 1] = fin.prior; o[t * 8 + 2] = fin.velo; o[t * 8 + 3] = ja ? 0.0 : fin.hand;
                    o[t * 8 + 4] = XT ? fin.face : 0.0; o[t * 8 + 5] = XT ? fin.shape : 0.0; o[t * 8 + 6] = XT ? fin.stay : 0.0; o[t * 8 + 7] = ja ? fin.hand : 0.0;
                }
                int* oi;
                if ((oi = chp->iters) != nullptr) { oi[t * 2 + 0] = n_iter; oi[t * 2 + 1] = n_fev; }
                if ((oi = chp->status) != nullptr) oi[t] = fail ? -1 : 0;
            }
        }
        __syncthreads();
        if (lead && rejoin_run > 0 && chp->abort_at != nullptr) {
            const int mark = __hip_atomic_load(chp->abort_at + chp->chunk0 + bi_next, __ATOMIC_RELAXED, __HIP_MEMORY_SCOPE_AGENT);
            if (chp->bnd_off + t < mark) rejoin_run = 0;
        }
        if (!COOP && rejoin_run >= 2 && t + 1 < F) { if (tid == 0 && chp->frames_done) *chp->frames_done = t + 1; break; }
        if (t + 1 == F && tid == 0 && lead && chp->frames_done) *chp->frames_done = F;
        PROF_ACC(19, _tr);
    }
    if constexpr (COOP) {
        if (cx.scal[S_COOP_FAIL] != 0.0 && lead && tid == 0 && chp->run_entry != nullptr) {
            const int S = 2 * NP + 5;
            chp->run_entry[(size_t)bi_next * S + 2 * NP + 3] = MOSHII_MARK_ENTRY_SPOILED;
            if (chp->abort_at != nullptr) chp->abort_at[chp->chunk0 + bi_next] = 0x7fffffff;
        }
        if (chp->baton != nullptr && cx.scal[S_COOP_FAIL] == 0.0) {
            __syncthreads();
            if (tid == 0) __threadfence();
            const unsigned seq = coop_begin(cx);
            const double mine[1] = {0.0};
            coop_exchange_small<1>(co, cx, seq, mine, cx.y);
            coop_end(cx, seq);
        }
    }
    if (lead && chp->baton != nullptr) {
        __syncthreads();
        if (tid == 0) {
            __threadfence();
            __hip_atomic_store(&chp->baton[2 * chp->chunk0], 2, __ATOMIC_RELEASE, __HIP_MEMORY_SCOPE_AGENT);
        }
    }
    if constexpr (!COOP && !XT) {
        if (chp->tail_done != nullptr) {
            (void)tail_cut;
            __syncthreads();
            if (tid == 0) { __threadfence(); atomicAdd(chp->tail_done, 1); }
        }
    }
    PROF_LAP(12);
#ifdef MOSHII_PROFILE
    if (threadIdx.x == 0 && blockIdx.x == 0) g_prof[30] += wall_clock64() - _wall0;
#endif
}

#ifdef MOSHII_DEV_ONLY_NBLK4
template __global__ void k_chain_solve<4, 1, false, false>(const ChainDev*, ModelDev, PriorDev, OptsDev, ChainLayout, int);
template __global__ void k_chain_solve<4, 1, false, true>(const ChainDev*, ModelDev, PriorDev, OptsDev, ChainLayout, int);
#else
#define MOSHII_INSTANTIATE(N, XT_, COOP_) \
    template __global__ void k_chain_solve<N, 1, XT_, COOP_>(const ChainDev*, ModelDev, PriorDev, OptsDev, ChainLayout, int);
MOSHII_INSTANTIATE(2, false, false)
MOSHII_INSTANTIATE(4, false, false)
MOSHII_INSTANTIATE(5, false, false)
MOSHII_INSTANTIATE(7, false, false)
MOSHII_INSTANTIATE(8, false, false)
MOSHII_INSTANTIATE(5, true, false)
MOSHII_INSTANTIATE(8, true, false)
MOSHII_INSTANTIATE(10, true, false)
MOSHII_INSTANTIATE(13, true, false)
MOSHII_INSTANTIATE(4, false, true)
MOSHII_INSTANTIATE(5, false, true)
MOSHII_INSTANTIATE(7, false, true)
MOSHII_INSTANTIATE(8, false, true)
MOSHII_INSTANTIATE(5, true, true)
MOSHII_INSTANTIATE(8, true, true)
MOSHII_INSTANTIATE(10, true, true)
MOSHII_INSTANTIATE(13, true, true)
#undef MOSHII_INSTANTIATE
#endif

__global__ __launch_bounds__(MOSHII_TPB) void k_markers(const AttachDev* __restrict__ attp, ModelDev md, ChainLayout ly,
                                                        const double* __restrict__ pose, const double* __restrict__ trans,
                                                        double* __restrict__ out) {
    extern __shared__ __attribute__((aligned(16))) double lds[];
    const int tid = threadIdx.x;
    const AttachDev at = *attp;
    const Ctx cx = make_ctx(lds, ly);
    const int f = blockIdx.x;
    for (int i = tid; i < md.NP; i += MOSHII_TPB) cx.pose[i] = pose[(size_t)f * md.NP + i];
    if (tid < 3) cx.trans[tid] = trans[(size_t)f * 3 + tid];
    __syncthreads();
    FrameParams fp;
    fp.obs = nullptr; fp.wt_data = 0.0; fp.wt_pose = 0.0; fp.wt_poseH = 0.0; fp.wt_velo = 0.0;
    fp.has_velo = 0; fp.use_fingers = 0; fp.nobs = 0;
    fp.wt_poseF = 0.0; fp.use_face = 0; fp.use_shape = 0; fp.has_stay = 0;
    PriorDev pr; pr.G = 0; pr.npose = 0; pr.means = nullptr; pr.chols = nullptr; pr.halfprec = nullptr; pr.neglogw = nullptr;
    OptsDev op;
    op.nbody = 0; op.nfinger = 0; op.n1 = 0; op.n2 = 0; op.maxiter = 0;
    op.step1 = nullptr; op.step2 = nullptr; op.body = nullptr; op.finger = nullptr;
    op.nface = 0; op.nshape = 0; op.face = nullptr;
    op.njangle = 0; op.wt_jangle = 0.0; op.jangle = nullptr;
    for (int k = 1 + tid; k < md.K; k += MOSHII_TPB) cx.ksum[k - 1] = k;
    for (int i = tid; i < 3 * md.K; i += MOSHII_TPB) cx.Jl[i] = md.J[i];
    __syncthreads();
    fp.v0 = 0; fp.v1 = 0;
    eval_forward<false>(cx, md, at, pr, op, cx.pose, cx.trans, fp, nullptr, cx.ksum, md.K - 1, at.vsh, false);
    for (int i = tid; i < 3 * at.M; i += MOSHII_TPB) out[(size_t)f * 3 * at.M + i] = cx.msim[i];
}

}

extern "C" hipError_t moshii_launch_chain_solve(int nblk, int xt, int n_chains, size_t lds_bytes, hipStream_t stream,
                                                const ChainDev* chains, const ModelDev* md, const PriorDev* pr,
                                                const OptsDev* op, const ChainLayout* ly, int coop_g) {
    using namespace moshii;
    void (*kern)(const ChainDev*, ModelDev, PriorDev, OptsDev, ChainLayout, int) = nullptr;
#ifdef MOSHII_DEV_ONLY_NBLK4
    if (xt || nblk != 4) return hipErrorInvalidValue;
    if (coop_g >= 1) kern = k_chain_solve<4, 1, false, true>; else kern = k_chain_solve<4, 1, false, false>;
// ... 62 lines not shown
```

### moshpp_amd/csrc/moshii_api.hip

```cpp
#include "../../include/moshii.h"
#include "moshii_dev.h"
#include "dev_mem.h"
#include "export_plan.h"
#include "solve_plan.h"
#include "stagei_views.h"

#include <algorithm>
#include <atomic>
#include <cmath>
#include <cstdio>
#include <cstdlib>
#include <cstring>
#include <memory>
#include <mutex>
#include <string>
#include <vector>

extern "C" hipError_t moshii_launch_chain_solve(int nblk, int xt, int n_chains, size_t lds_bytes, hipStream_t stream,
                                                const ChainDev* chains, const ModelDev* md, const PriorDev* pr,
                                                const OptsDev* op, const ChainLayout* ly, int coop_g);
extern "C" hipError_t moshii_launch_markers(int F, size_t lds_bytes, hipStream_t stream, const AttachDev* att,
                                            const ModelDev* md, const ChainLayout* ly, const double* pose,
                                            const double* trans, double* out);
extern "C" hipError_t moshii_launch_lbs_f32(hipStream_t stream, const ModelDev* md, int F, const float* pose,
// ... 1105 lines not shown
        if (g == 0) return 0;
    }
    if (g == 1) return 0;
    if (g < 0 || g > MOSHII_COOP_MAXG) return -2;
    return g;
}

struct SolveDims { int xt, nshape, nmax, nblk, nkfmax, nhj, G, npose; };

int check_opts(moshii_model_t m, moshii_prior_t prior, const moshii_solve_opts* o, SolveDims* d) {
    if (!m->betas_set) return fail(MOSHII_ERR_ARG, "moshii_model_set_betas has not been called");
    if (o->n_body > 0 && (!prior || prior->npose != o->n_body)) return fail(MOSHII_ERR_ARG, "prior npose must equal n_body");
    if (o->n_step1 < 0 || o->n_step2 < 0 || o->n_step1 > m->NP || o->n_step2 > m->NP) return fail(MOSHII_ERR_ARG, "bad free-variable lists");
    const int NP = m->NP;
    const int nshape = o->n_shape;
    if (nshape < 0 || o->n_face < 0) return fail(MOSHII_ERR_ARG, "bad Step-2 extras");
    if (nshape > 0 && nshape != m->nshape) return fail(MOSHII_ERR_ARG, "n_shape must equal the block of moshii_model_set_free_shape");
    if (o->n_face > 0 && !o->face_ids) return fail(MOSHII_ERR_ARG, "face_ids missing");
    for (int i = 1; i < o->n_face; ++i)
        if (o->face_ids[i] != o->face_ids[i - 1] + 1) return fail(MOSHII_ERR_UNSUPPORTED, "face ids must be contiguous");
    if (o->n_jangle < 0 || (o->n_jangle > 0 && !o->jangle_ids)) return fail(MOSHII_ERR_ARG, "bad joint-angle term");
    for (int i = 0; i < o->n_jangle; ++i)
        if (o->jangle_ids[i] < 0 || o->jangle_ids[i] >= NP) return fail(MOSHII_ERR_ARG, "joint-angle id out of range");
    if (o->n_jangle > 0 && o->n_finger > 0)
        return fail(MOSHII_ERR_UNSUPPORTED, "a joint-angle term and finger ids in one solve (no SMAL model has fingers)");
    const int xt = (nshape > 0 || o->n_face > 0) ? 1 : 0;
    const int nmax = 3 + std::max(o->n_step1, o->n_step2 + nshape);
    int nblk = pick_nblk(nmax, xt != 0);
    if (nblk < 0) return fail(MOSHII_ERR_UNSUPPORTED, xt ? "more than 207 unknowns per step" : "more than 124 free pose variables per step");
    if (const char* e = getenv("MOSHII_FORCE_NBLK")) nblk = std::max(nblk, atoi(e));
    auto count_kf = [&](const int32_t* ids, int n) {
        std::vector<char> need(m->K, 0);
        for (int i = 0; i < n; ++i) {
            if (ids[i] < 0 || ids[i] >= NP) return -1;
            if (ids[i] < m->body_dof) need[ids[i] / 3] = 1;
            else for (int k = m->body_dof / 3; k < m->K; ++k) need[k] = 1;
        }
        int c = 0; for (char b : need) c += b; return c;
    };
    const int kf1 = count_kf(o->step1_ids, o->n_step1), kf2 = count_kf(o->step2_ids, o->n_step2);
    if (kf1 < 0 || kf2 < 0) return fail(MOSHII_ERR_ARG, "free pose id out of range");
    if (o->n_finger > 0)
        for (int i = 1; i < o->n_finger; ++i)
            if (o->finger_ids[i] != o->finger_ids[i - 1] + 1) return fail(MOSHII_ERR_UNSUPPORTED, "finger ids must be contiguous");
    bool hand_free = false;
    for (int i = 0; i < o->n_step1; ++i) hand_free |= o->step1_ids[i] >= m->body_dof;
    for (int i = 0; i < o->n_step2; ++i) hand_free |= o->step2_ids[i] >= m->body_dof;
    d->xt = xt; d->nshape = nshape; d->nmax = nmax; d->nblk = nblk;
    d->nkfmax = std::max(1, std::max(kf1, kf2));
    d->nhj = hand_free ? (m->K - m->body_dof / 3) : 0;
    d->G = prior ? prior->G : 0; d->npose = prior ? prior->npose : 0;
    return MOSHII_OK;
}

int choose_layout(moshii_model_t m, const SolveDims& d, int Mmax, int Nvmax, int NWmax, int n_workgroups, int coop_g, LaunchCfg* cfg) {
    const int xt = d.xt, nmax = d.nmax, npose = d.npose;
    int nblk = d.nblk;
    auto layout = [&](int Tm) { return make_layout(m, Mmax, Nvmax, NWmax, npose, d.G, nmax, d.nkfmax, Tm, nblk, d.nhj, d.nshape); };
    const int n_cu = cu_count();
    int budget = 160 * 1024;
    if (const char* e = getenv("MOSHII_LDS_BUDGET")) budget = atoi(e);
    int Tm;
    ChainLayout ly;
    if (coop_g == -1) coop_g = solve_plan::own_group_size(Mmax, d.nkfmax, npose > 0, !xt && nblk < 4);
    if (coop_g > 0 && ((!xt && nmax + 1 > 8 * 16) || (long long)coop_g * std::max(n_workgroups, 1) > n_cu)) coop_g = 0;
    if (coop_g > 0) {
        if (!xt && nblk < 4) nblk = 4;
        if (nmax + 1 > nblk * 16) return fail(MOSHII_ERR_UNSUPPORTED, "cooperative chains: too many unknowns");
        if (coop_g > MOSHII_COOP_MAXG) return fail(MOSHII_ERR_ARG, "cooperative chains: at most 8 workgroups per chain");
        cfg->coop_prior_frac = (npose > 0) ? ((coop_g >= 3) ? (xt ? 0.5 : 0.0) : 0.4) : 1.0;
        if (const char* e = getenv("MOSHII_COOP_PRIOR_FRAC")) cfg->coop_prior_frac = std::min(1.0, std::max(0.0, atof(e)));
        int mlo[MOSHII_COOP_MAXG + 1];
        coop_split(Mmax, coop_g, cfg->coop_prior_frac, mlo);
        int share = 2;
        for (int r = 0; r < coop_g; ++r) share = std::max(share, mlo[r + 1] - mlo[r]);
        Tm = std::min(40, share + 1);
        ly = layout(Tm);
        while (Tm > 2 && (size_t)ly.total_doubles * 8 > (size_t)budget) ly = layout(--Tm);
        cfg->coop = CoopLayout(nblk, Mmax, coop_g);
        cfg->coop_prior_rank = coop_g - 1;
    } else
    if (const char* e = getenv("MOSHII_TM")) {
        Tm = std::max(1, std::min(40, atoi(e)));
        ly = layout(Tm);
    } else {
        int best = -1, best_cost = 0;
        for (int t = std::min(40, std::max(2, Mmax)); t >= 2; --t) {
            const ChainLayout lt = layout(t);
            if ((size_t)lt.total_doubles * 8 > (size_t)budget) continue;
            const int full = Mmax / t, rem = Mmax % t;
            const int rounds = full * ((t * d.nkfmax + 255) / 256) + (rem ? (rem * d.nkfmax + 255) / 256 : 0);
            const int cost = 3 * rounds + 4 * (full + (rem ? 1 : 0));
            if (best < 0 || cost < best_cost) { best = t; best_cost = cost; }
        }
        if (best < 0) best = 2;
        Tm = best;
        ly = layout(Tm);
    }
    const size_t lds_bytes = (size_t)ly.total_doubles * sizeof(double);
    if (lds_bytes > 160 * 1024) return fail(MOSHII_ERR_UNSUPPORTED, "problem does not fit the 160 KiB LDS of a CU");
    cfg->nblk = nblk; cfg->xt = xt; cfg->ly = ly; cfg->lds_bytes = lds_bytes;
    cfg->coop_g = coop_g;
    return MOSHII_OK;
}

int upload_ids(moshii_model_t m, moshii_prior_t prior, const moshii_solve_opts* o, hipStream_t stream, size_t extra_bytes, LaunchCfg* cfg,
               size_t* ctl_off) {
    const int nshape = o->n_shape, njangle = std::max(0, o->n_jangle);
    const size_t nids = (size_t)o->n_step1 + o->n_step2 + o->n_body + o->n_finger + o->n_face + njangle;
    const size_t need = sizeof(int) * (nids + 16) + 64 + extra_bytes;
    int rc = m->scratch.reserve(need, stream);
    if (rc) return rc;
    std::vector<int> ids;
    ids.reserve(nids);
    const size_t e1 = 0, e2 = e1 + o->n_step1, eb = e2 + o->n_step2, ef = eb + o->n_body;
    ids.insert(ids.end(), o->step1_ids, o->step1_ids + o->n_step1);
    ids.insert(ids.end(), o->step2_ids, o->step2_ids + o->n_step2);
    ids.insert(ids.end(), o->body_ids, o->body_ids + o->n_body);
    ids.insert(ids.end(), o->finger_ids, o->finger_ids + o->n_finger);
    const size_t efc = ids.size();
    ids.insert(ids.end(), o->face_ids, o->face_ids + o->n_face);
    const size_t eja = ids.size();
    if (njangle > 0) ids.insert(ids.end(), o->jangle_ids, o->jangle_ids + njangle);
    char* dbase = m->scratch.ptr;
    if (!ids.empty()) {
        HIP_TRY(hipMemcpyAsync(dbase, ids.data(), ids.size() * sizeof(int), hipMemcpyHostToDevice, stream));
        HIP_TRY(hipStreamSynchronize(stream));
    }
    *ctl_off = (ids.size() * sizeof(int) + 63) & ~size_t(63);

    OptsDev& od = cfg->od;
    od.wt_data = o->wt_data; od.wt_velo = o->wt_velo; od.wt_poseB = o->wt_poseB; od.wt_poseH = o->wt_poseH;
    od.wt_annealing = o->wt_annealing; od.num_train_markers = o->num_train_markers;
    od.e3_first = o->e3_first; od.e3 = o->e3; od.delta0 = o->delta0; od.maxiter = o->maxiter;
    od.n1 = o->n_step1; od.n2 = o->n_step2; od.nbody = o->n_body; od.nfinger = o->n_finger;
    od.same_sets = (nshape == 0 && o->n_step1 == o->n_step2 && std::equal(o->step1_ids, o->step1_ids + o->n_step1, o->step2_ids)) ? 1 : 0;
    od.wt_poseF = o->wt_poseF; od.wt_shape = o->wt_shape; od.wt_shape_stay = o->wt_shape_stay;
    od.nface = o->n_face; od.nshape = nshape;
    const int* dids = (const int*)dbase;
    od.step1 = as_gp(dids + e1); od.step2 = as_gp(dids + e2); od.body = as_gp(dids + eb); od.finger = as_gp(dids + ef); od.face = as_gp(dids + efc);
    od.njangle = njangle; od.wt_jangle = njangle > 0 ? o->wt_jangle : 0.0; od.jangle = as_gp(dids + eja);
    memset(&cfg->pd, 0, sizeof(cfg->pd));
    if (prior) cfg->pd = prior->dev();
    cfg->md = m->dev();
    return MOSHII_OK;
}

int prepare_launch(moshii_model_t m, moshii_prior_t prior, const moshii_solve_opts* o, int Mmax, int Nvmax, int NWmax,
                   int n_workgroups, hipStream_t stream, size_t extra_bytes, LaunchCfg* cfg, size_t* ctl_off, int coop_g = 0) {
    SolveDims d;
    int rc;
    if ((rc = check_opts(m, prior, o, &d))) return rc;
    if ((rc = choose_layout(m, d, Mmax, Nvmax, NWmax, n_workgroups, coop_g, cfg))) return rc;
    return upload_ids(m, prior, o, stream, extra_bytes, cfg, ctl_off);
}

int launch_chains(const LaunchCfg& cfg, int n, const ChainDev* d_chains, hipStream_t stream) {
    HIP_TRY(moshii_launch_chain_solve(cfg.nblk, cfg.xt, n, cfg.lds_bytes, stream, d_chains, &cfg.md, &cfg.pd, &cfg.od, &cfg.ly, cfg.coop_g));
    note_launch("k_chain_solve<" + std::to_string(cfg.nblk) + ",1" + (cfg.xt ? ",xt" : "") +
                (cfg.coop_g > 0 ? ",coop" + std::to_string(cfg.coop_g) : "") + ">", (int)cfg.lds_bytes, MOSHII_TPB);
    return MOSHII_OK;
}

size_t qscratch_bytes(const LaunchCfg& cfg, int K, int E) {
    const size_t nfac = (cfg.nblk > 8) ? (size_t)(cfg.ly.nmax + 1) * (cfg.ly.nmax + 2) / 2 + 12 + 256 : 0;
    return ((size_t)2 * K * E * 3 + nfac) * sizeof(double);
}

int reserve_exchange(moshii_model_t m, const CoopLayout& cl, size_t n_chains, hipStream_t stream) {
    int rc = m->coopbuf.reserve(cl.bytes_per_chain * n_chains, stream);
    if (rc) return rc;
    HIP_TRY(hipMemsetAsync(m->coopbuf.ptr, 0, cl.bytes_per_chain * n_chains, stream));
    return MOSHII_OK;
}

void fill_coop(ChainDev& cd, const LaunchCfg& cfg, int M, char* slice) {
    cd.coop.G = cfg.coop_g; cd.coop.prior_rank = cfg.coop_prior_rank; cd.coop.slot_doubles = cfg.coop.slot_doubles; cd.coop.skew = coop_skew_env();
    coop_split(M, cfg.coop_g, cfg.coop_prior_frac, cd.coop.mlo);
    cd.coop.slots = as_gp_rw((unsigned long long*)slice);
    cd.coop.flags = as_gp_rw((unsigned*)(slice + cfg.coop.flags_offset));
}

int coop_any_broken(moshii_model_t m, const CoopLayout& cl, size_t n_chains, hipStream_t stream, bool* broken) {
    std::vector<unsigned> ab(n_chains, 0u);
    HIP_TRY(hipMemcpy2DAsync(ab.data(), sizeof(unsigned), m->coopbuf.ptr + cl.abort_offset, cl.bytes_per_chain, sizeof(unsigned), n_chains,
                             hipMemcpyDeviceToHost, stream));
    HIP_TRY(hipStreamSynchronize(stream));
    *broken = false;
    for (unsigned a : ab) *broken |= a != 0u;
    return MOSHII_OK;
}

struct FrameBufs {
    int F, M;
    const double* obs; const uint8_t* vis;
    double *pose, *fullpose, *trans, *msim, *errs; int *iters, *status;
    double* shape;
};
struct Staged {
    FrameBufs rows = {};
    DevArena mem;
};
struct CallBufs {
    std::vector<Staged> st;
    DevArena mem;
    explicit CallBufs(size_t n) : st(n) {}
};

int stage_in(const FrameBufs& h, int NP, int P, size_t n_shape, hipStream_t stream, Staged* s) {
    const size_t Fz = std::max(h.F, 1), M = h.M;
    FrameBufs& d = s->rows;
    d.F = h.F; d.M = h.M;
    DevArena& mem = s->mem;
    d.obs = mem.upload(h.obs, (size_t)h.F * M * 3);
    d.vis = mem.upload(h.vis, (size_t)h.F * M);
    d.pose = mem.zeros<double>(Fz * NP, stream);
    d.fullpose = mem.zeros<double>(Fz * P, stream);
    d.trans = mem.zeros<double>(Fz * 3, stream);
    d.msim = mem.zeros<double>(Fz * M * 3, stream);
    d.errs = mem.zeros<double>(Fz * MOSHII_NERR, stream);
    d.iters = mem.zeros<int>(Fz * 2, stream);
    d.status = mem.zeros<int>(Fz, stream);
    if (n_shape > 0) d.shape = mem.zeros<double>(n_shape, stream);
    return mem.ok() ? MOSHII_OK : fail_mem(mem, "staging a chain's frames");
}

int stage_out(const FrameBufs& h, int NP, int P, int E, const Staged& s) {
    const size_t F = h.F, M = h.M;
    const FrameBufs& d = s.rows;
    if (!F) return MOSHII_OK;
    if (h.pose) HIP_TRY(hipMemcpy(h.pose, d.pose, F * NP * sizeof(double), hipMemcpyDeviceToHost));
    if (h.fullpose) HIP_TRY(hipMemcpy(h.fullpose, d.fullpose, F * P * sizeof(double), hipMemcpyDeviceToHost));
    if (h.trans) HIP_TRY(hipMemcpy(h.trans, d.trans, F * 3 * sizeof(double), hipMemcpyDeviceToHost));
    if (h.msim) HIP_TRY(hipMemcpy(h.msim, d.msim, F * M * 3 * sizeof(double), hipMemcpyDeviceToHost));
    if (h.errs) HIP_TRY(hipMemcpy(h.errs, d.errs, F * MOSHII_NERR * sizeof(double), hipMemcpyDeviceToHost));
    if (h.iters) HIP_TRY(hipMemcpy(h.iters, d.iters, F * 2 * sizeof(int), hipMemcpyDeviceToHost));
    if (h.status) HIP_TRY(hipMemcpy(h.status, d.status, F * sizeof(int), hipMemcpyDeviceToHost));
    if (h.shape && d.shape) HIP_TRY(hipMemcpy(h.shape, d.shape, F * E * sizeof(double), hipMemcpyDeviceToHost));
    return MOSHII_OK;
}

__global__ void k_verify_chunks(int n, int NP, int E, const int* __restrict__ pred, const double* __restrict__ entry,
                                const double* __restrict__ fin, double* __restrict__ dev) {
    const int c = blockIdx.x;
    if (c >= n) return;
    const int p = pred[c];
    __shared__ double red[64];
    double d = 0.0;
    if (p >= 0) {
        const int S = 2 * NP + 5 + E;
        const double* a = entry + (size_t)c * S;
        const double* b = fin + (size_t)p * S;
        const bool flags_ok = (a[2 * NP + 3] == b[2 * NP + 3]) && (a[2 * NP + 4] == b[2 * NP + 4]);
        const bool hp = a[2 * NP + 3] != 0.0;
        bool nan = false;
        for (int i = threadIdx.x; i < 2 * NP + 3; i += blockDim.x) {
            if (i >= NP && i < 2 * NP && !hp) continue;
            const double v = fabs(a[i] - b[i]);
            nan |= !(v == v);
            d = fmax(d, v);
        }
        for (int e = threadIdx.x; e < E; e += blockDim.x) {
            const double v = fabs(a[2 * NP + 5 + e] - b[2 * NP + 5 + e]);
            nan |= !(v == v);
            d = fmax(d, v);
        }
        if (nan) d = MOSHII_HANDOFF_NAN;
        else if (a[2 * NP + 3] == MOSHII_MARK_ENTRY_SPOILED && b[2 * NP + 3] != MOSHII_MARK_FINAL_SPOILED) d = MOSHII_HANDOFF_GIVEN_UP;
        else if (b[2 * NP + 3] == MOSHII_MARK_FINAL_SPOILED) d = MOSHII_HANDOFF_PRED_GIVEN_UP;
        else if (!flags_ok) d = MOSHII_HANDOFF_MISMATCH;
    }
    red[threadIdx.x] = d;
    __syncthreads();
    for (int o = 32; o > 0; o >>= 1) { if ((int)threadIdx.x < o) red[threadIdx.x] = fmax(red[threadIdx.x], red[threadIdx.x + o]); __syncthreads(); }
    if (threadIdx.x == 0) dev[c] = red[0];
}

int chain_solve_once(moshii_model_t m, moshii_prior_t prior, const moshii_solve_opts* o, int32_t n_chains, const moshii_chain_desc* chains,
                     uint32_t flags, hipStream_t stream, bool* broken) {
    *broken = false;
    const bool dev = (flags & MOSHII_BUFFERS_DEVICE) != 0;
    const int NP = m->NP, P = m->P;
    int Mmax = 0, Nvmax = 0, NWmax = 1;
    for (int c = 0; c < n_chains; ++c) {
        const moshii_chain_desc& ch = chains[c];
        if (!ch.attach || ch.attach->model != m || ch.F < 0 || !ch.obs || !ch.vis) return fail(MOSHII_ERR_ARG, "bad chain descriptor");
        Mmax = std::max(Mmax, ch.attach->M); Nvmax = std::max(Nvmax, ch.attach->Nv); NWmax = std::max(NWmax, ch.attach->NW);
    }
    const int E = o->n_shape > 0 ? o->n_shape : 0;
    const size_t extra = sizeof(ChainDev) * n_chains + sizeof(double) * (size_t)n_chains * (2 * NP + 4 + E + 2) + 256;
    int coop_req = coop_request(flags, "MOSHII_COOP");
    if (coop_req < -1) return fail(MOSHII_ERR_ARG, "cooperative chains: group size out of range");
    LaunchCfg cfg;
    size_t ctl = 0;
    int rc = prepare_launch(m, prior, o, Mmax, Nvmax, NWmax, n_chains, stream, extra, &cfg, &ctl, coop_req);
    if (rc) return rc;
    const int coop_g = cfg.coop_g;
    if (coop_g > 0 && (rc = reserve_exchange(m, cfg.coop, n_chains, stream))) return rc;
    char* dbase = m->scratch.ptr + ctl;
    const size_t qbytes = qscratch_bytes(cfg, m->K, E);
    const int qranks = (coop_g > 0) ? coop_g : 1;
    if (E > 0 && (rc = m->qscratch.reserve(qbytes * n_chains * qranks, stream))) return rc;
    std::vector<char> hostbuf(extra, 0);
    size_t off = sizeof(ChainDev) * n_chains;
    auto put = [&](const void* src, size_t bytes) { off = (off + 15) & ~size_t(15); size_t o2 = off; memcpy(hostbuf.data() + off, src, bytes); off += bytes; return o2; };
    CallBufs bufs(dev ? 0 : n_chains);
// ... 411 lines not shown
```

### moshpp_amd/csrc/moshii_dev.h

```cpp
#pragma once
#include <hip/hip_runtime.h>
#include <stdint.h>
#include "solve_plan.h"

#define MOSHII_MAXK 64

#ifndef MOSHII_AS_GLOBAL
#define MOSHII_AS_GLOBAL __attribute__((address_space(1)))
#endif
template <class T> __device__ __forceinline__ const T MOSHII_AS_GLOBAL* gptr(const T* p) { return (const T MOSHII_AS_GLOBAL*)p; }
template <class T> __device__ __forceinline__ T MOSHII_AS_GLOBAL* gptr(T* p) { return (T MOSHII_AS_GLOBAL*)p; }
#if defined(__HIP_DEVICE_COMPILE__)
template <class T> __device__ __forceinline__ const T MOSHII_AS_GLOBAL* gptr(const T MOSHII_AS_GLOBAL* p) { return p; }
#endif
#if defined(__HIP_DEVICE_COMPILE__)
#define MOSHII_GP(T) T MOSHII_AS_GLOBAL*
#else
#define MOSHII_GP(T) T*
#endif
template <class T> __host__ __device__ inline MOSHII_GP(const T) as_gp(const T* p) { return (MOSHII_GP(const T))p; }
template <class T> __host__ __device__ inline MOSHII_GP(T) as_gp_rw(T* p) { return (MOSHII_GP(T))p; }
#define MOSHII_TPB 256

struct ModelDev {
    int V, K, P, NP, body_dof, hand_dof, nhand_full, maxdepth;
    MOSHII_GP(const int) parents;
    MOSHII_GP(const double) J;
    MOSHII_GP(const double) hands_mean;
    MOSHII_GP(const double) comps;
    MOSHII_GP(const int) comp_lo;
    MOSHII_GP(const int) comp_hi;
    MOSHII_GP(const int) col_lo;
    MOSHII_GP(const int) col_hi;
    MOSHII_GP(const unsigned long long) anc;
    MOSHII_GP(const int) depth;
    int nshape;
    MOSHII_GP(const double) JS;
};

struct AttachDev {
    int M, Nv, Nvp, NW;
    MOSHII_GP(const double) vsh;
    MOSHII_GP(const double) Pt;
    MOSHII_GP(const double) Pj;
    MOSHII_GP(const int) wj;
    MOSHII_GP(const double) ww;
    MOSHII_GP(const double) coef;
    MOSHII_GP(const double) Ssh;
};

struct PriorDev {
    int G, npose;
    MOSHII_GP(const double) means;
    MOSHII_GP(const double) chols;
    MOSHII_GP(const double) halfprec;
    MOSHII_GP(const double) neglogw;
    MOSHII_GP(const double) cnorm;
};

struct OptsDev {
    double wt_data, wt_velo, wt_poseB, wt_poseH, wt_annealing, num_train_markers;
    double e3_first, e3, delta0;
    int maxiter, n1, n2, nbody, nfinger, same_sets;
    MOSHII_GP(const int) step1;
    MOSHII_GP(const int) step2;
    MOSHII_GP(const int) body;
    MOSHII_GP(const int) finger;
    double wt_poseF, wt_shape, wt_shape_stay;
    int nface, nshape;
    MOSHII_GP(const int) face;
    int njangle;
    double wt_jangle;
    MOSHII_GP(const int) jangle;
};

#define MOSHII_COOP_MAXG 8
struct CoopDev {
    int G;
    int prior_rank;
    int mlo[MOSHII_COOP_MAXG + 1];
    int slot_doubles;
    int qstride;
    int skew;
    MOSHII_GP(unsigned long long) slots;
    MOSHII_GP(unsigned int) flags;
};
struct CoopCtx {
    int G, rank, prior_rank, mlo, mhi, slot_doubles, skew;
    int prior_bare;
    MOSHII_GP(unsigned long long) slots;
    MOSHII_GP(unsigned int) flags;
};

struct ChainDev {
    const AttachDev* att;
    int F, first;
    const double* obs;
    const uint8_t* vis;
    const double* init_pose;
    const double* init_trans;
    const double* init_prev;
    double* pose;
    double* fullpose;
    double* trans;
    double* msim;
    double* errs;
    int* iters;
    int* status;
    int skip;
    const double* init_state;
    double* entry_state;
    double* final_state;
    int nb;
    const int* bnd;
    double* run_final;
    double* run_entry;
    int* frames_done;
    int* baton;
    int* abort_at;
    int chunk0;
    int bnd_off;
    const double* init_shape;
    double* shape;
    double* qscratch;
    double rejoin_tol;
    int fuse_F;
    int fuse_c;
    int fuse_has_next;
    int fuse_has_prev;
    int* fuse_flags;
    int* fuse_count;
    double fuse_tol;
    CoopDev coop;
    int* tail_done;
    int tail_quota, tail_left;
    int tail_can_cut;
    int* tail_mark;
};

struct ChainLayout {
    int Mmax, Nvmax, NWmax, nmax, Tm, nkfmax, LDJ, nhj;
    int NPX;
    int o_vshp, o_shp0;
    int o_pose, o_trans, o_pose_t, o_trans_t, o_pose_prev, o_vtarget, o_fullpose;
    int o_feat, o_B, o_omega, o_Rw, o_tw, o_Rloc, o_acol, o_Jl;
    int o_vposed, o_vpos, o_msim, o_res, o_vconst;
    int o_xb, o_ell, o_score;
    int o_px0, o_ps0;
    int o_g, o_dsd, o_dgn, o_ddl, o_y;
    int o_red, o_scal;
    int o_anc;
    int o_ints;
    int o_big;
    int big_doubles;
    int total_doubles;
    int i_visidx, i_colpid, i_colprior, i_pid2prior, i_jointslot, i_kfree, i_colq, i_ksum, i_kconst, i_total;
    int t_Jh, t_Jrow, t_Lm, t_Trot, t_xjs, t_rest, t_tjs;
};

struct KernelCtx {
    ChainLayout ly;
    ModelDev md;
    PriorDev pr;
    OptsDev op;
    AttachDev at;
    double fp_raw[12];
    CoopCtx co;
    unsigned long long kargs;
};
#define MOSHII_KC_DOUBLES ((int)((sizeof(KernelCtx) + 15) / 16 * 2))

struct Lbs32Model {
    float* v_shaped;
    float* posedirs_t;
    float* weights;
    float* J;
    float* hcompf;
    float* hmeanf;
    float* jtab;
    float* hcj;
    int jtab_valid;
    int* varflag;
    int epoch;
    int Vp;
    _Float16* Pfrag;
    int* perm;
    char* tables;
    unsigned tab_gnr;
    unsigned tab_gjid;
    unsigned tab_gx;
    unsigned tab_vshs;
    unsigned tab_vsc;
    unsigned tab_gw;
    long long* dbgbuf;
    int K, NRM;
    float pscale, inv_pscale;
    int NVT, KS;
    int KJ;
    int mfma_ok;
    float* Atr;
    _Float16* featF;
    int Fcap;
    _Float16* PfragX;
    float* JSf;
    float* Sft;
    int nshape, KSX;
    float sxscale;
    long long featcap;
};

struct RenderVertex {
    int sx, sy;
    double z;
    float n[3];
    int ok;
};
struct RenderMarker {
    double uc, vc;
    double rx, ry;
    float depth;
    int ok;
};
struct RenderArgs {
    int V, NF, N, W, H, w16;
    const unsigned* tris;
    const RenderVertex* rec;
    const RenderMarker* mrec;
    const unsigned char* prgb;
    unsigned char body[3], bg[3];
    double ambient;
    unsigned char* rgb;
    int* ids;
    float* depth;
};
```

Measured before the change: 66240.

## Outline cold chain-solve phases into noinline functions with a slim body context

Moves rarely executed per-frame work (marker gathering, rigid init, column tables, posedirs constants, chunk boundary and fuse handoff logic) out of the main solve loop into noinline device functions that rebuild their context from LDS. It also introduces a smaller BodyCtx whose control-vector pointers are derived from fixed LDJ offsets, plus a host-side check that the layout satisfies those offsets. The goal is to shrink register pressure and code size in the hot loop, at the cost of call overhead and reloading context in the cold paths.

```diff
diff --git a/moshpp_amd/csrc/chain_solve.hip b/moshpp_amd/csrc/chain_solve.hip
--- a/moshpp_amd/csrc/chain_solve.hip
+++ b/moshpp_amd/csrc/chain_solve.hip
@@ -3,8 +3,10 @@
 #include <type_traits>
 #if defined(__HIP_DEVICE_COMPILE__)
 #define MOSHII_OPAQUE(x) __asm__ __volatile__("" : "+v"(x))
+#define MOSHII_OPAQUE_S(x) __asm__ __volatile__("" : "+s"(x))
 #else
 #define MOSHII_OPAQUE(x) do {} while (0)
+#define MOSHII_OPAQUE_S(x) do {} while (0)
 #endif
 __device__ __forceinline__ double uni64(double v) {
 #if defined(__HIP_DEVICE_COMPILE__)
@@ -59,6 +61,28 @@
     int* tjs;
 };
 
+struct BodyCtx {
+    double *pose, *trans, *pose_t, *trans_t, *pose_prev, *vtarget, *fullpose, *msim;
+    double *g, *dsd, *dgn, *ddl, *y, *red, *scal;
+    int *visidx, *colpid, *colprior, *colq;
+};
+template <int NBLK>
+__device__ __forceinline__ BodyCtx make_body_ctx(double* lds, const ChainLayout& ly) {
+    constexpr int LDJ = 16 * NBLK;
+    auto at = [&](int off) { MOSHII_OPAQUE_S(off); return lds + off; };
+    BodyCtx cx;
+    cx.pose = at(ly.o_pose); cx.trans = at(ly.o_trans); cx.pose_t = at(ly.o_pose_t); cx.trans_t = at(ly.o_trans_t);
+    cx.pose_prev = at(ly.o_pose_prev); cx.vtarget = at(ly.o_vtarget); cx.fullpose = at(ly.o_fullpose); cx.msim = at(ly.o_msim);
+    double* ctl = at(ly.o_g);
+    cx.g = ctl; cx.dsd = ctl + LDJ; cx.dgn = ctl + 2 * LDJ; cx.ddl = ctl + 3 * LDJ; cx.y = ctl + 4 * LDJ;
+    cx.red = ctl + 5 * LDJ; cx.scal = ctl + 5 * LDJ + 16;
+    int* ints = reinterpret_cast<int*>(at(ly.o_ints));
+    auto iat = [&](int off) { MOSHII_OPAQUE_S(off); return ints + off; };
+    cx.visidx = iat(ly.i_visidx); cx.colq = iat(ly.i_colq);
+    cx.colpid = iat(ly.i_colpid); cx.colprior = cx.colpid + LDJ;
+    return cx;
+}
+
 struct FrameParams {
     const double* obs;
     double wt_data, wt_pose, wt_poseH, wt_velo;
@@ -224,7 +248,8 @@
 #endif
     return __hip_atomic_load(p, __ATOMIC_RELAXED, __HIP_MEMORY_SCOPE_AGENT);
 }
-__device__ __forceinline__ unsigned coop_begin(const Ctx& cx) { return (unsigned)__builtin_amdgcn_readfirstlane((int)cx.scal[S_COOP_SEQ]) + 1u; }
+template <class C>
+__device__ __forceinline__ unsigned coop_begin(const C& cx) { return (unsigned)__builtin_amdgcn_readfirstlane((int)cx.scal[S_COOP_SEQ]) + 1u; }
 __device__ __forceinline__ MOSHII_GP(unsigned long long) coop_slot(const CoopCtx& co, unsigned seq, int r) {
     return co.slots + ((size_t)(seq & 1u) * co.G + r) * co.slot_doubles;
 }
@@ -266,8 +291,8 @@
         for (unsigned i = h & 3u; i > 0u; --i) __builtin_amdgcn_s_sleep(127);
     }
 }
-template <bool L2 = false>
-__device__ __forceinline__ bool coop_publish_wait(const CoopCtx& co, const Ctx& cx, unsigned seq) {
+template <bool L2 = false, class C>
+__device__ __forceinline__ bool coop_publish_wait(const CoopCtx& co, const C& cx, unsigned seq) {
     const int tid = threadIdx.x;
     coop_skew(co, seq);
     PROF_T(_tp0);
@@ -302,13 +327,14 @@
     TRACE_STAMP(co, seq, 2);
     return cx.scal[S_COOP_FAIL] == 0.0;
 }
-__device__ __forceinline__ void coop_end(const Ctx& cx, unsigned seq) {
+template <class C>
+__device__ __forceinline__ void coop_end(const C& cx, unsigned seq) {
     __syncthreads();
     if (threadIdx.x == 0) cx.scal[S_COOP_SEQ] = (double)seq;
     __syncthreads();
 }
-template <int NS, bool L2>
-__device__ __forceinline__ bool coop_exchange_small_(const CoopCtx& co, const Ctx& cx, unsigned seq, const double (&mine)[NS], double* land) {
+template <int NS, bool L2, class C>
+__device__ __forceinline__ bool coop_exchange_small_(const CoopCtx& co, const C& cx, unsigned seq, const double (&mine)[NS], double* land) {
     const int tid = threadIdx.x;
     const int goff = co.slot_doubles - 32;
     coop_skew(co, seq);
@@ -342,8 +368,8 @@
     TRACE_STAMP(co, seq, 2);
     return cx.scal[S_COOP_FAIL] == 0.0;
 }
-template <int NS>
-__device__ __forceinline__ bool coop_exchange_small(const CoopCtx& co, const Ctx& cx, unsigned seq, const double (&mine)[NS], double* land) {
+template <int NS, class C>
+__device__ __forceinline__ bool coop_exchange_small(const CoopCtx& co, const C& cx, unsigned seq, const double (&mine)[NS], double* land) {
     return coop_exchange_small_<NS, false>(co, cx, seq, mine, land);
 }
 
@@ -2266,6 +2292,13 @@
 #else
 #define MOSHII_CTX_FROM_KARGS(kc) const ChainLayout ly = uniform_load(&(kc)->ly); const ModelDev md = uniform_load(&(kc)->md); const PriorDev pr = uniform_load(&(kc)->pr); const OptsDev op = uniform_load(&(kc)->op);
 #endif
+#if defined(__HIP_DEVICE_COMPILE__) && !defined(MOSHII_NO_KARGS)
+typedef KArgsPtr BodyArgs;
+__device__ __forceinline__ BodyArgs body_args(const KernelCtx* kc) { return kargs_of(kc); }
+#else
+typedef const KernelCtx* BodyArgs;
+__device__ __forceinline__ BodyArgs body_args(const KernelCtx* kc) { return kc; }
+#endif
 
 template <int NBLK>
 __device__ __noinline__ bool coop_rs_reduce(unsigned seq_) {
@@ -2426,67 +2459,408 @@
     for (int i = 0; i < 3; ++i) cx.trans[i] = bm[i] - (R[i * 3 + 0] * am[0] + R[i * 3 + 1] * am[1] + R[i * 3 + 2] * am[2]);
 }
 
+template <class T>
+__device__ __forceinline__ T* uniform_ptr(T* p) {
+    const unsigned long long v = (unsigned long long)p;
+    return (T*)(((unsigned long long)(unsigned)__builtin_amdgcn_readfirstlane((int)(v >> 32)) << 32) | (unsigned)__builtin_amdgcn_readfirstlane((int)v));
+}
+
+__device__ __noinline__ void coop_gather_markers_fn() {
+    extern __shared__ __attribute__((aligned(16))) double lds[];
+    const KernelCtx* kc = reinterpret_cast<const KernelCtx*>(lds);
+    MOSHII_CTX_FROM_KARGS(kc)
+    const AttachDev at = uniform_load(&kc->at);
+    const Ctx cx = make_ctx(lds, ly);
+    const CoopCtx co = uniform_load(&kc->co);
+    const int tid = threadIdx.x;
+    {
+        const unsigned seq = coop_begin(cx);
+        auto gather = [&](auto l2) {
+            constexpr bool L2 = decltype(l2)::value;
+            auto* mine = coop_slot(co, seq, co.rank);
+            for (int i = 3 * co.mlo + tid; i < 3 * co.mhi; i += MOSHII_TPB) coop_st64<L2>(mine + i, f64_bits(cx.msim[i]));
+            if (tid == 0) coop_st64<L2>(mine + 3 * at.M, f64_bits((double)co.mlo));
+            if (coop_publish_wait<L2>(co, cx, seq)) {
+                const int M3 = 3 * at.M;
+                for (int i = tid; i < M3; i += MOSHII_TPB) {
+                    int r = 0;
+                    for (int q = 1; q < co.G; ++q) r += (i >= 3 * (int)bits_f64(coop_ld64<L2>(coop_slot(co, seq, q) + 3 * at.M))) ? 1 : 0;
+                    if (r != co.rank) cx.msim[i] = bits_f64(coop_ld64<L2>(coop_slot(co, seq, r) + i));
+                }
+            }
+        };
+        gather(std::false_type());
+        coop_end(cx, seq);
+    }
+}
+template <bool XT, bool COOP>
+__device__ __noinline__ void rigid_init_fn(const uint8_t* visrow) {
+    extern __shared__ __attribute__((aligned(16))) double lds[];
+    const KernelCtx* kc = reinterpret_cast<const KernelCtx*>(lds);
+    MOSHII_CTX_FROM_KARGS(kc)
+    const AttachDev at = uniform_load(&kc->at);
+    const FrameParams fp = uniform_load(reinterpret_cast<const FrameParams*>(kc->fp_raw));
+    const Ctx cx = make_ctx(lds, ly);
+    const int tid = threadIdx.x;
+    const int NPX = XT ? ly.NPX : md.NP;
+    if constexpr (COOP) coop_gather_markers_fn();
+    if (tid == 0) rigid_init_serial(cx, fp, visrow, at.M);
+    __syncthreads();
+    for (int i = tid; i < NPX; i += MOSHII_TPB) cx.pose_t[i] = cx.pose[i];
+    if (tid < 3) cx.trans_t[tid] = cx.trans[tid];
+    __syncthreads();
+}
+
+template <bool XT>
+__device__ __noinline__ void column_tables_fn(int step2_) {
+    extern __shared__ __attribute__((aligned(16))) double lds[];
+    const KernelCtx* kc = reinterpret_cast<const KernelCtx*>(lds);
+    MOSHII_CTX_FROM_KARGS(kc)
+    const Ctx cx = make_ctx(lds, ly);
+    const int tid = threadIdx.x;
+    const bool step2 = __builtin_amdgcn_readfirstlane(step2_) != 0;
+    const auto ids = step2 ? op.step2 : op.step1;
+    const int nids = step2 ? op.n2 : op.n1, nshp = (XT && step2) ? op.nshape : 0;
+    const int ncp = 3 + nids;
+    const int n = ncp + (XT ? nshp : 0);
+    for (int i = tid; i < md.NP; i += MOSHII_TPB) cx.colq[i] = -1;
+    __syncthreads();
+    for (int q = tid; q < n; q += MOSHII_TPB) {
+        const int pid = (q < 3) ? -1 : ((q < ncp) ? ids[q - 3] : md.NP + (q - ncp));
+        cx.colpid[q] = pid;
+        cx.colprior[q] = (pid >= 0 && pid < md.NP) ? cx.pid2prior[pid] : -1;
+        if (pid >= 0 && pid < md.NP) cx.colq[pid] = q;
+    }
+    if (tid == 0) {
+        for (int k = 0; k < md.K; ++k) cx.jointslot[k] = -1;
+        for (int i = 0; i < nids; ++i) {
+            const int pid = ids[i];
+            if (pid < md.body_dof) cx.jointslot[pid / 3] = 0;
+            else for (int k = md.body_dof / 3; k < md.K; ++k) cx.jointslot[k] = 0;
+        }
+        int c = 0;
+        for (int k = 0; k < md.K; ++k) if (cx.jointslot[k] == 0) { cx.jointslot[k] = c; cx.kfree[c] = k; ++c; }
+        cx.scal[S_TMP0] = (double)c;
+        int nh = 0;
+        for (int i = 0; i < nids; ++i) nh += (ids[i] >= md.body_dof) ? 1 : 0;
+        cx.scal[S_TMP2] = (double)nh;
+        int ns = 0, nc = 0;
+        for (int k = 1; k < md.K; ++k) { if (cx.jointslot[k] >= 0) cx.ksum[ns++] = k; else cx.kconst[nc++] = k; }
+        cx.scal[S_TMP3] = (double)ns;
+    }
+    __syncthreads();
+}
+
+template <bool COOP>
+__device__ __noinline__ void vconst_fn(int nkc_) {
+    extern __shared__ __attribute__((aligned(16))) double lds[];
+    const KernelCtx* kc = reinterpret_cast<const KernelCtx*>(lds);
+    MOSHII_CTX_FROM_KARGS(kc)
+    const AttachDev at = uniform_load(&kc->at);
+    const Ctx cx = make_ctx(lds, ly);
+    CoopCtx co = CoopCtx();
+    if constexpr (COOP) co = uniform_load(&kc->co);
+    const int tid = threadIdx.x;
+    const int nkc = __builtin_amdgcn_readfirstlane(nkc_);
+    for (int d = tid; d < md.P; d += MOSHII_TPB) cx.fullpose[d] = fullpose_entry(md, cx.pose, d);
+    __syncthreads();
+    if (tid < md.K) {
+        double R[9];
+        rodrigues_R(&cx.fullpose[3 * tid], R);
+#pragma unroll
+        for (int e = 0; e < 9; ++e) cx.feat[tid * 9 + e] = R[e] - ((e == 0 || e == 4 || e == 8) ? 1.0 : 0.0);
+    }
+    __syncthreads();
+    if constexpr (COOP) posedirs_partial_range(cx, at, cx.kconst, nkc, at.vsh, cx.vconst, 3 * co.mlo, 3 * co.mhi);
+    else posedirs_partial(cx, at, cx.kconst, nkc, at.vsh, cx.vconst);
+    __syncthreads();
+}
+
+__device__ __noinline__ int coop_lead_verdict_fn(const ChainDev* chp_, int t_, int rejoin_run_, int bi_next_, int st_) {
+    extern __shared__ __attribute__((aligned(16))) double lds[];
+    const KernelCtx* kc = reinterpret_cast<const KernelCtx*>(lds);
+    MOSHII_CTX_FROM_KARGS(kc)
+    const Ctx cx = make_ctx(lds, ly);
+    const int tid = threadIdx.x;
+    const ChainDev* chp = uniform_ptr(chp_);
+    const int t = __builtin_amdgcn_readfirstlane(t_), rejoin_run = __builtin_amdgcn_readfirstlane(rejoin_run_), stf = __builtin_amdgcn_readfirstlane(st_);
+    int bi_next = __builtin_amdgcn_readfirstlane(bi_next_);
+    const bool has_prev = (stf & 1) != 0, first = (stf & 2) != 0;
+    const int NP = md.NP, F = chp->F;
+    bool halt = false;
+    const int S = 2 * NP + 5;
+    if (rejoin_run >= 2 && t < F) {
+        if (tid == 0 && chp->frames_done) *chp->frames_done = t;
+        halt = true;
+    }
+    if (!halt && bi_next < chp->nb && t == chp->bnd[bi_next] - chp->bnd_off) {
+        double* s1 = chp->run_final + (size_t)bi_next * S;
+        for (int i = tid; i < NP; i += MOSHII_TPB) { s1[i] = cx.pose[i]; s1[NP + i] = cx.pose_prev[i]; }
+        if (tid < 3) s1[2 * NP + tid] = cx.trans[tid];
+        if (tid == 3) s1[2 * NP + 3] = has_prev ? 1.0 : 0.0;
+        if (tid == 4) s1[2 * NP + 4] = first ? 1.0 : 0.0;
+        if (chp->baton != nullptr) {
+            if (tid == 0) {
+                int* st = chp->baton + 2 * (chp->chunk0 + 1 + bi_next);
+                double go = 1.0;
+                if (__hip_atomic_load(st, __ATOMIC_ACQUIRE, __HIP_MEMORY_SCOPE_AGENT) == 1) {
+                    __hip_atomic_store(st + 1, 1, __ATOMIC_RELEASE, __HIP_MEMORY_SCOPE_AGENT);
+                    int spins = 0;
+                    while (__hip_atomic_load(st, __ATOMIC_ACQUIRE, __HIP_MEMORY_SCOPE_AGENT) != 2) {
+                        __builtin_amdgcn_s_sleep(64);
+                        if (++spins > 20000) { go = 0.0; break; }
+                    }
+                }
+                __builtin_amdgcn_fence(__ATOMIC_ACQUIRE, "agent");
+                cx.scal[S_BATON] = go;
+            }
+            __syncthreads();
+            if (cx.scal[S_BATON] == 0.0) { if (tid == 0 && chp->frames_done) *chp->frames_done = t; halt = true; }
+            __syncthreads();
+        }
+        if (!halt) {
+            double* s2 = chp->run_entry + (size_t)(bi_next + 1) * S;
+            for (int i = tid; i < NP; i += MOSHII_TPB) { s2[i] = cx.pose[i]; s2[NP + i] = cx.pose_prev[i]; }
+            if (tid < 3) s2[2 * NP + tid] = cx.trans[tid];
+            if (tid == 3) s2[2 * NP + 3] = has_prev ? 1.0 : 0.0;
+            if (tid == 4) s2[2 * NP + 4] = first ? 1.0 : 0.0;
+            ++bi_next;
+        }
+    }
+    if (!halt && chp->baton != nullptr && t < F) {
+        if (tid == 0) cx.scal[S_ABORT] = (double)__hip_atomic_load(&chp->baton[2 * chp->chunk0 + 1], __ATOMIC_RELAXED, __HIP_MEMORY_SCOPE_AGENT);
+        __syncthreads();
+        if (cx.scal[S_ABORT] != 0.0) {
+            if (tid == 0) {
+                chp->run_entry[(size_t)bi_next * S + 2 * NP + 3] = MOSHII_MARK_ENTRY_SPOILED;
+                int* mark = chp->abort_at + chp->chunk0 + bi_next;
+                if (*mark < chp->bnd_off + t) *mark = chp->bnd_off + t;
+                if (chp->frames_done) *chp->frames_done = -t - 1;
+            }
+            halt = true;
+        }
+        __syncthreads();
+    }
+    return (bi_next << 1) | (halt ? 1 : 0);
+}
+
+template <bool XT>
+__device__ __noinline__ int carry_on_fn(const ChainDev* chp_, int t_, int st_) {
+    extern __shared__ __attribute__((aligned(16))) double lds[];
+    const KernelCtx* kc = reinterpret_cast<const KernelCtx*>(lds);
+    MOSHII_CTX_FROM_KARGS(kc)
+    const Ctx cx = make_ctx(lds, ly);
+    const int tid = threadIdx.x;
+    const ChainDev* chp = uniform_ptr(chp_);
+    const int t = __builtin_amdgcn_readfirstlane(t_), stf = __builtin_amdgcn_readfirstlane(st_);
+    const bool has_prev = (stf & 1) != 0, first = (stf & 2) != 0;
+    const int NP = md.NP, F = chp->F, skip = chp->skip;
+    const int S = 2 * NP + 5 + (XT ? op.nshape : 0);
+    if (t == skip && chp->entry_state != nullptr) {
+        __syncthreads();
+        if (tid == 0) { __threadfence(); __hip_atomic_store(&chp->fuse_flags[3 * chp->fuse_c], 1, __ATOMIC_RELEASE, __HIP_MEMORY_SCOPE_AGENT); }
+    }
+    if (chp->fuse_F == 0 && t == F) {
+        __syncthreads();
+        if (tid == 0) {
+            __threadfence();
+            __hip_atomic_store(&chp->fuse_flags[3 * chp->fuse_c + 1], 1, __ATOMIC_RELEASE, __HIP_MEMORY_SCOPE_AGENT);
+            __hip_atomic_store(&chp->fuse_flags[3 * chp->fuse_c + 2], 1, __ATOMIC_RELEASE, __HIP_MEMORY_SCOPE_AGENT);
+        }
+    }
+    if (chp->fuse_F > 0 && t == chp->fuse_F) {
+        double* sf = chp->run_final - S;
+        for (int i = tid; i < NP; i += MOSHII_TPB) { sf[i] = cx.pose[i]; sf[NP + i] = cx.pose_prev[i]; }
+        if (tid < 3) sf[2 * NP + tid] = cx.trans[tid];
+        if (tid == 3) sf[2 * NP + 3] = has_prev ? 1.0 : 0.0;
+        if (tid == 4) sf[2 * NP + 4] = first ? 1.0 : 0.0;
+        if constexpr (XT) for (int e = tid; e < op.nshape; e += MOSHII_TPB) sf[2 * NP + 5 + e] = cx.pose[NP + e];
+        __syncthreads();
+        if (tid == 0) { __threadfence(); __hip_atomic_store(&chp->fuse_flags[3 * chp->fuse_c + 1], 1, __ATOMIC_RELEASE, __HIP_MEMORY_SCOPE_AGENT); }
+        bool carry = false;
+        auto state_dev = [&](const double* en) {
+            double dv = 0.0, nn = 0.0;
+            for (int i = tid; i < NP; i += MOSHII_TPB) { dv = fmax(dv, fmax(fabs(cx.pose[i] - en[i]), fabs(cx.pose_prev[i] - en[NP + i]))); nn += en[i] + en[NP + i]; }
+            if (tid < 3) dv = fmax(dv, fabs(cx.trans[tid] - en[2 * NP + tid]));
+            if (tid == 3 && (has_prev ? 1.0 : 0.0) != en[2 * NP + 3]) dv = MOSHII_HANDOFF_MISMATCH;
+            if (tid == 4 && (first ? 1.0 : 0.0) != en[2 * NP + 4]) dv = MOSHII_HANDOFF_MISMATCH;
+            if constexpr (XT) for (int e = tid; e < op.nshape; e += MOSHII_TPB) dv = fmax(dv, fabs(cx.pose[NP + e] - en[2 * NP + 5 + e]));
+            if (!(nn == nn)) dv = MOSHII_HANDOFF_MISMATCH;
+            return block_max(dv, cx.red);
+        };
+        auto wait_flag = [&](int* fl, int patience) {
+            if (tid == 0) {
+                double go = 1.0;
+                int spins = 0;
+                while (__hip_atomic_load(fl, __ATOMIC_ACQUIRE, __HIP_MEMORY_SCOPE_AGENT) != 1) {
+                    __builtin_amdgcn_s_sleep(64);
+                    if (++spins > patience) { go = 0.0; break; }
+                }
+                __builtin_amdgcn_fence(__ATOMIC_ACQUIRE, "agent");
+                cx.scal[S_BATON] = go;
+            }
+            __syncthreads();
+            const bool ok_ = cx.scal[S_BATON] != 0.0;
+            __syncthreads();
+            return ok_;
+        };
+        if (chp->fuse_has_next && wait_flag(chp->fuse_flags + 3 * (chp->fuse_c + 1), 2000)) {
+            const double dv = state_dev(chp->run_entry);
+            carry = !(dv <= chp->fuse_tol);
+            if (carry && dv > 1e-6 && chp->fuse_has_prev && wait_flag(chp->fuse_flags + 3 * (chp->fuse_c - 1) + 1, 150)) {
+                const double* lf = chp->run_final - 2 * S;
+                const double* oe = chp->run_entry - S;
+                double dl = 0.0;
+                for (int i = tid; i < 2 * NP + 3; i += MOSHII_TPB) dl = fmax(dl, fabs(lf[i] - oe[i]));
+                dl = block_max(dl, cx.red);
+                if (!(dl <= 1e-6)) carry = false;
+            }
+        }
+        if (carry && tid == 0) __hip_atomic_store(&chp->baton[2 * chp->chunk0], 1, __ATOMIC_RELEASE, __HIP_MEMORY_SCOPE_AGENT);
+        __syncthreads();
+        if (tid == 0) { __threadfence(); __hip_atomic_store(&chp->fuse_flags[3 * chp->fuse_c + 2], 1, __ATOMIC_RELEASE, __HIP_MEMORY_SCOPE_AGENT); }
+        if (!carry) { if (tid == 0 && chp->frames_done) *chp->frames_done = t; return 1; }
+        if (tid == 0) {
+            int* fl = chp->fuse_flags + 3 * (chp->fuse_c + 1) + 1;
+            double go = 1.0;
+            int spins = 0;
+            while (__hip_atomic_load(fl, __ATOMIC_ACQUIRE, __HIP_MEMORY_SCOPE_AGENT) != 1 ||
+                   __hip_atomic_load(fl + 1, __ATOMIC_ACQUIRE, __HIP_MEMORY_SCOPE_AGENT) != 1) {
+                if (__hip_atomic_load(&chp->baton[2 * chp->chunk0 + 1], __ATOMIC_RELAXED, __HIP_MEMORY_SCOPE_AGENT) != 0) { go = 0.0; break; }
+                __builtin_amdgcn_s_sleep(64);
+                if (++spins > 20000) { go = 0.0; break; }
+            }
+            __builtin_amdgcn_fence(__ATOMIC_ACQUIRE, "agent");
+            if (go != 0.0 && chp->fuse_count != nullptr) atomicAdd(chp->fuse_count, 1);
+            cx.scal[S_BATON] = go;
+        }
+        __syncthreads();
+        if (cx.scal[S_BATON] == 0.0) { if (tid == 0 && chp->frames_done) *chp->frames_done = t; return 1; }
+        double* s2 = chp->run_entry;
+        for (int i = tid; i < NP; i += MOSHII_TPB) { s2[i] = cx.pose[i]; s2[NP + i] = cx.pose_prev[i]; }
+        if (tid < 3) s2[2 * NP + tid] = cx.trans[tid];
+        if (tid == 3) s2[2 * NP + 3] = has_prev ? 1.0 : 0.0;
+        if (tid == 4) s2[2 * NP + 4] = first ? 1.0 : 0.0;
+        if constexpr (XT) for (int e = tid; e < op.nshape; e += MOSHII_TPB) s2[2 * NP + 5 + e] = cx.pose[NP + e];
+        return 2;
+    }
+    return 0;
+}
+
+template <bool XT>
+__device__ __noinline__ int chunk_boundary_fn(const ChainDev* chp_, int t_, int bi_next_, int st_) {
+    extern __shared__ __attribute__((aligned(16))) double lds[];
+    const KernelCtx* kc = reinterpret_cast<const KernelCtx*>(lds);
+    MOSHII_CTX_FROM_KARGS(kc)
+    const Ctx cx = make_ctx(lds, ly);
+    const int tid = threadIdx.x;
+    const ChainDev* chp = uniform_ptr(chp_);
+    const int t = __builtin_amdgcn_readfirstlane(t_), bi_next = __builtin_amdgcn_readfirstlane(bi_next_), stf = __builtin_amdgcn_readfirstlane(st_);
+    const bool has_prev = (stf & 1) != 0, first = (stf & 2) != 0;
+    const int NP = md.NP;
+    const int S = 2 * NP + 5 + (XT ? op.nshape : 0);
+    double* s1 = chp->run_final + (size_t)bi_next * S;
+    for (int i = tid; i < NP; i += MOSHII_TPB) { s1[i] = cx.pose[i]; s1[NP + i] = cx.pose_prev[i]; }
+    if (tid < 3) s1[2 * NP + tid] = cx.trans[tid];
+    if (tid == 3) s1[2 * NP + 3] = has_prev ? 1.0 : 0.0;
+    if (tid == 4) s1[2 * NP + 4] = first ? 1.0 : 0.0;
+    if constexpr (XT) for (int e = tid; e < op.nshape; e += MOSHII_TPB) s1[2 * NP + 5 + e] = cx.pose[NP + e];
+    if (chp->baton != nullptr) {
+        if (tid == 0) {
+            int* st = chp->baton + 2 * (chp->chunk0 + 1 + bi_next);
+            double go = 1.0;
+            if (chp->fuse_flags != nullptr) {
+                int* vd = chp->fuse_flags + 3 * (chp->chunk0 + bi_next) + 2;
+                int spins = 0;
+                while (__hip_atomic_load(vd, __ATOMIC_ACQUIRE, __HIP_MEMORY_SCOPE_AGENT) != 1) {
+                    __builtin_amdgcn_s_sleep(64);
+                    if (++spins > 20000) { go = 0.0; break; }
+                }
+            }
+            if (go != 0.0 && __hip_atomic_load(st, __ATOMIC_ACQUIRE, __HIP_MEMORY_SCOPE_AGENT) == 1) {
+                __hip_atomic_store(st + 1, 1, __ATOMIC_RELEASE, __HIP_MEMORY_SCOPE_AGENT);
+                int spins = 0;
+                while (__hip_atomic_load(st, __ATOMIC_ACQUIRE, __HIP_MEMORY_SCOPE_AGENT) != 2) {
+                    __builtin_amdgcn_s_sleep(64);
+                    if (++spins > 20000) { go = 0.0; break; }
+                }
+            }
+            if (go != 0.0 && chp->fuse_flags != nullptr) {
+                int* od = chp->fuse_flags + 3 * (chp->chunk0 + 1 + bi_next) + 1;
+                int spins = 0;
+                while (__hip_atomic_load(od, __ATOMIC_ACQUIRE, __HIP_MEMORY_SCOPE_AGENT) != 1) {
+                    __builtin_amdgcn_s_sleep(64);
+                    if (++spins > 20000) { go = 0.0; break; }
+                }
+            }
+            __builtin_amdgcn_fence(__ATOMIC_ACQUIRE, "agent");
+            cx.scal[S_BATON] = go;
+        }
+        __syncthreads();
+        if (cx.scal[S_BATON] == 0.0) { if (tid == 0 && chp->frames_done) *chp->frames_done = t; return 0; }
+    }
+    double* s2 = chp->run_entry + (size_t)(bi_next + 1) * S;
+    for (int i = tid; i < NP; i += MOSHII_TPB) { s2[i] = cx.pose[i]; s2[NP + i] = cx.pose_prev[i]; }
+    if (tid < 3) s2[2 * NP + tid] = cx.trans[tid];
+    if (tid == 3) s2[2 * NP + 3] = has_prev ? 1.0 : 0.0;
+    if (tid == 4) s2[2 * NP + 4] = first ? 1.0 : 0.0;
+    if constexpr (XT) for (int e = tid; e < op.nshape; e += MOSHII_TPB) s2[2 * NP + 5 + e] = cx.pose[NP + e];
+    return 1;
+}
+
+template <bool XT>
+__device__ __noinline__ int territory_request_fn(const ChainDev* chp_, int t_, int bi_next_) {
+    extern __shared__ __attribute__((aligned(16))) double lds[];
+    const KernelCtx* kc = reinterpret_cast<const KernelCtx*>(lds);
+    MOSHII_CTX_FROM_KARGS(kc)
+    double* scal = lds + ly.o_scal;
+    const int tid = threadIdx.x;
+    const ChainDev* chp = uniform_ptr(chp_);
+    const int t = __builtin_amdgcn_readfirstlane(t_), bi_next = __builtin_amdgcn_readfirstlane(bi_next_);
+    const int NP = md.NP;
+    if (tid == 0) scal[S_ABORT] = (double)__hip_atomic_load(&chp->baton[2 * chp->chunk0 + 1], __ATOMIC_RELAXED, __HIP_MEMORY_SCOPE_AGENT);
+    __syncthreads();
+    if (scal[S_ABORT] != 0.0) {
+        if (tid == 0) {
+            const int S = 2 * NP + 5 + (XT ? op.nshape : 0);
+            chp->run_entry[(size_t)bi_next * S + 2 * NP + 3] = MOSHII_MARK_ENTRY_SPOILED;
+            int* mark = chp->abort_at + chp->chunk0 + bi_next;
+            if (*mark < chp->bnd_off + t) *mark = chp->bnd_off + t;
+            if (chp->frames_done) *chp->frames_done = -t - 1;
+        }
+        return 1;
+    }
+    return 0;
+}
+
 template <int NBLK, bool XT, bool COOP>
-__device__ Sse run_phase(const Ctx& cx, const ChainLayout& ly, const ModelDev& md, const AttachDev& at, const PriorDev& pr,
-                         const OptsDev& op, const FrameParams& fp, const uint8_t* visrow, MOSHII_GP(const int) ids, int nids, int nshp,
+__device__ Sse run_phase(const BodyCtx& cx, const FrameParams& fp,
+                         const uint8_t* visrow, bool step2, int nids, int nshp,
                          double* qs, double e3,
                          bool rigid, bool eval_only, bool reuse, Sse& carried, bool& at_pose, int& fwd_set, int set_id, int& vc_key,
                          int& tab_key, int& n_iter, int& n_fev, int& fail, const CoopCtx& co) {
+    extern __shared__ __attribute__((aligned(16))) double lds[];
     const int tid = threadIdx.x;
     const int ncp = 3 + nids;
     const int n = ncp + (XT ? nshp : 0);
-    const int NPX = XT ? ly.NPX : md.NP;
+    const BodyArgs ka = body_args(reinterpret_cast<const KernelCtx*>(lds));
+    const int NPX = XT ? ka->ly.NPX : ka->md.NP;
+    const int i_ksum = ka->ly.i_ksum, o_vconst = ka->ly.o_vconst, o_big = ka->ly.o_big, maxiter = ka->op.maxiter;
+    const int o_pose = (int)(cx.pose - lds), o_pose_t = (int)(cx.pose_t - lds), o_trans_t = (int)(cx.trans_t - lds), o_g = (int)(cx.g - lds);
     if (!eval_only && tab_key != set_id) {
         tab_key = set_id;
-        for (int i = tid; i < md.NP; i += MOSHII_TPB) cx.colq[i] = -1;
-        __syncthreads();
-        for (int q = tid; q < n; q += MOSHII_TPB) {
-            const int pid = (q < 3) ? -1 : ((q < ncp) ? ids[q - 3] : md.NP + (q - ncp));
-            cx.colpid[q] = pid;
-            cx.colprior[q] = (pid >= 0 && pid < md.NP) ? cx.pid2prior[pid] : -1;
-            if (pid >= 0 && pid < md.NP) cx.colq[pid] = q;
-        }
-        if (tid == 0) {
-            for (int k = 0; k < md.K; ++k) cx.jointslot[k] = -1;
-            for (int i = 0; i < nids; ++i) {
-                const int pid = ids[i];
-                if (pid < md.body_dof) cx.jointslot[pid / 3] = 0;
-                else for (int k = md.body_dof / 3; k < md.K; ++k) cx.jointslot[k] = 0;
-            }
-            int c = 0;
-            for (int k = 0; k < md.K; ++k) if (cx.jointslot[k] == 0) { cx.jointslot[k] = c; cx.kfree[c] = k; ++c; }
-            cx.scal[S_TMP0] = (double)c;
-            int nh = 0;
-            for (int i = 0; i < nids; ++i) nh += (ids[i] >= md.body_dof) ? 1 : 0;
-            cx.scal[S_TMP2] = (double)nh;
-            int ns = 0, nc = 0;
-            for (int k = 1; k < md.K; ++k) { if (cx.jointslot[k] >= 0) cx.ksum[ns++] = k; else cx.kconst[nc++] = k; }
-            cx.scal[S_TMP3] = (double)ns;
-        }
-        __syncthreads();
+        column_tables_fn<XT>(step2 ? 1 : 0);
     }
     const int nkf = (int)cx.scal[S_TMP0], nfree_hand = (int)cx.scal[S_TMP2];
     const int nks = (int)cx.scal[S_TMP3];
-    const int nkc = md.K - 1 - nks;
+    const int nkc = ka->md.K - 1 - nks;
     if (vc_key != set_id) {
-        for (int d = tid; d < md.P; d += MOSHII_TPB) cx.fullpose[d] = fullpose_entry(md, cx.pose, d);
-        __syncthreads();
-        if (tid < md.K) {
-            double R[9];
-            rodrigues_R(&cx.fullpose[3 * tid], R);
-#pragma unroll
-            for (int e = 0; e < 9; ++e) cx.feat[tid * 9 + e] = R[e] - ((e == 0 || e == 4 || e == 8) ? 1.0 : 0.0);
-        }
-        __syncthreads();
-        if constexpr (COOP) posedirs_partial_range(cx, at, cx.kconst, nkc, at.vsh, cx.vconst, 3 * co.mlo, 3 * co.mhi);
-        else posedirs_partial(cx, at, cx.kconst, nkc, at.vsh, cx.vconst);
-        __syncthreads();
+        vconst_fn<COOP>(nkc);
         vc_key = set_id;
     }
     AReg<NBLK> A;
     A.zero();
     if (tid == 0) {
-        extern __shared__ __attribute__((aligned(16))) double lds[];
         static_assert(sizeof(FrameParams) <= sizeof(KernelCtx::fp_raw), "KernelCtx::fp_raw too small");
         *reinterpret_cast<FrameParams*>(reinterpret_cast<KernelCtx*>(lds)->fp_raw) = fp;
     }
@@ -2494,7 +2868,7 @@
     if (tid < 3) cx.trans_t[tid] = cx.trans[tid];
     __syncthreads();
     Sse last;
-    double sse = 0.0, delta = op.delta0, norm_sd = 0.0, norm_gn = 0.0, step = 0.0, p2 = 0.0, gd = 0.0;
+    double sse = 0.0, delta = ka->op.delta0, norm_sd = 0.0, norm_gn = 0.0, step = 0.0, p2 = 0.0, gd = 0.0;
     double dAd = 0.0, dl_dd = 0.0, dl_gs = 0.0, dl_ds = 0.0;
     bool init = true, done = false, have_gn = false;
     int iteration = 0;
@@ -2503,37 +2877,14 @@
     while (true) {
         int tid = threadIdx.x; MOSHII_OPAQUE(tid);
         if (skip_eval) { last = carried; skip_eval = false; }
-        else { PROF_T(_te); last = eval_forward_fn<XT, COOP>(visrow, ly.o_pose_t, ly.o_trans_t, ly.i_ksum, nks, ly.o_vconst, light); PROF_ACC(15, _te); }
+        else { PROF_T(_te); last = eval_forward_fn<XT, COOP>(visrow, o_pose_t, o_trans_t, i_ksum, nks, o_vconst, light); PROF_ACC(15, _te); }
         if constexpr (COOP) { if (cx.scal[S_COOP_FAIL] != 0.0) break; }
         if (!(last.total == last.total)) { fail = 1; break; }
         light = 0;
         at_pose = true;
         fwd_set = set_id;
         if (rigid) {
-            if constexpr (COOP) {
-                const unsigned seq = coop_begin(cx);
-                auto gather = [&](auto l2) {
-                    constexpr bool L2 = decltype(l2)::value;
-                    auto* mine = coop_slot(co, seq, co.rank);
-                    for (int i = 3 * co.mlo + tid; i < 3 * co.mhi; i += MOSHII_TPB) coop_st64<L2>(mine + i, f64_bits(cx.msim[i]));
-                    if (tid == 0) coop_st64<L2>(mine + 3 * at.M, f64_bits((double)co.mlo));
-                    if (coop_publish_wait<L2>(co, cx, seq)) {
-                        const int M3 = 3 * at.M;
-                        for (int i = tid; i < M3; i += MOSHII_TPB) {
-                            int r = 0;
-                            for (int q = 1; q < co.G; ++q) r += (i >= 3 * (int)bits_f64(coop_ld64<L2>(coop_slot(co, seq, q) + 3 * at.M))) ? 1 : 0;
-                            if (r != co.rank) cx.msim[i] = bits_f64(coop_ld64<L2>(coop_slot(co, seq, r) + i));
-                        }
-                    }
-                };
-                gather(std::false_type());
-                coop_end(cx, seq);
-            }
-            if (tid == 0) rigid_init_serial(cx, fp, visrow, at.M);
-            __syncthreads();
-            for (int i = tid; i < NPX; i += MOSHII_TPB) cx.pose_t[i] = cx.pose[i];
-            if (tid < 3) cx.trans_t[tid] = cx.trans[tid];
-            __syncthreads();
+            rigid_init_fn<XT, COOP>(visrow);
             rigid = false;
             continue;
         }
@@ -2561,7 +2912,7 @@
         PROF_ACC(23, _t1);
         double pp = 0.0, gg = 0.0, gAg = 0.0;
         if (do_assemble) {
-            { PROF_T(_ta); A = APass<NBLK, MOSHII_ASM_RET_VEC(NBLK)>::unpack(assemble_fn<NBLK, XT, COOP>(ly.o_pose, n, ncp, nkf, nfree_hand, qs)); PROF_ACC(16, _ta); }
+            { PROF_T(_ta); A = APass<NBLK, MOSHII_ASM_RET_VEC(NBLK)>::unpack(assemble_fn<NBLK, XT, COOP>(o_pose, n, ncp, nkf, nfree_hand, qs)); PROF_ACC(16, _ta); }
             if constexpr (COOP) { if (cx.scal[S_COOP_FAIL] != 0.0) break; }
             PROF_T(_t2);
             double gm = 0.0;
@@ -2585,7 +2936,7 @@
             if (delta <= 1e-15 * sqrt(pnorm2)) done = true;
         }
         if (init || improved) {
-            if (!init && iteration >= op.maxiter) done = true;
+            if (!init && iteration >= maxiter) done = true;
             if (done) break;
             ++iteration;
             const double csd = gg / gAg;
@@ -2607,8 +2958,8 @@
                 constexpr bool BIG = XT && NBLK > 8;
                 bool solved;
                 PROF_T(_ts);
-                if constexpr (BIG) solved = ldl_big<NBLK>(A, qs + (size_t)6 * md.K * op.nshape, cx.big, cx.g, cx.dgn, cx.y, n);
-                else solved = ldl_solve<NBLK>(A, ly.o_big, ly.o_g, ly.o_dgn, ly.o_y, n);
+                if constexpr (BIG) solved = ldl_big<NBLK>(A, qs + (size_t)6 * ka->md.K * ka->op.nshape, lds + o_big, cx.g, cx.dgn, cx.y, n);
+                else solved = ldl_solve<NBLK>(A, o_big, o_g, o_g + 2 * 16 * NBLK, o_g + 4 * 16 * NBLK, n);
                 PROF_ACC(17, _ts);
                 PROF_ACC(26, _t4);
                 if (!solved) {
@@ -2665,8 +3016,8 @@
 
 
 template <int NBLK, int MINW, bool XT, bool COOP = false>
-__global__ __launch_bounds__(MOSHII_TPB, MINW) void k_chain_solve(const ChainDev* __restrict__ chains, ModelDev md, PriorDev pr,
-                                                             OptsDev op, ChainLayout ly, int n_chains) {
+__global__ __launch_bounds__(MOSHII_TPB, MINW) void k_chain_solve(const ChainDev* __restrict__ chains, ModelDev a_md, PriorDev a_pr,
+                                                             OptsDev a_op, ChainLayout a_ly, int n_chains) {
     extern __shared__ __attribute__((aligned(16))) double lds[];
     const int tid = threadIdx.x;
     int chain_id = blockIdx.x;
@@ -2685,16 +3036,16 @@
     const bool lead = !COOP || co.rank == 0;
     const ChainDev* chp = chains + chain_id;
     const AttachDev at = *chp->att;
-    const Ctx cx = make_ctx(lds, ly);
+    const BodyCtx cx = make_body_ctx<NBLK>(lds, a_ly);
     if (tid == 0) {
         KernelCtx* kc = reinterpret_cast<KernelCtx*>(lds);
-        kc->ly = ly; kc->md = md; kc->pr = pr; kc->op = op; kc->at = at;
+        kc->ly = a_ly; kc->md = a_md; kc->pr = a_pr; kc->op = a_op; kc->at = at;
 #if defined(__HIP_DEVICE_COMPILE__)
         kc->kargs = (unsigned long long)__builtin_amdgcn_kernarg_segment_ptr();
 #if !defined(MOSHII_NO_KARGS)
         {
             const KArgsPtr kk = (KArgsPtr)__builtin_amdgcn_kernarg_segment_ptr();
-            if (kk->chains != chains || kk->n_chains != n_chains || kk->ly.total_doubles != ly.total_doubles || kk->md.V != md.V || kk->op.maxiter != op.maxiter)
+            if (kk->chains != chains || kk->n_chains != n_chains || kk->ly.total_doubles != a_ly.total_doubles || kk->md.V != a_md.V || kk->op.maxiter != a_op.maxiter)
                 __builtin_trap();
         }
 #endif
@@ -2702,9 +3053,10 @@
         if constexpr (COOP) { kc->co = co; cx.scal[S_COOP_SEQ] = 0.0; cx.scal[S_COOP_FAIL] = 0.0; }
     }
 
-    const int NP = md.NP, M = at.M, F = chp->F, skip = chp->skip;
+    const int NP = a_md.NP, M = at.M, F = chp->F, skip = chp->skip;
     bool has_prev, first;
     {
+        const Ctx cs = make_ctx(lds, a_ly);
         const double* is = chp->init_state;
         const double* ip = chp->init_pose;
         const double* iv = chp->init_prev;
@@ -2713,23 +3065,23 @@
             cx.pose[i] = is ? is[i] : (ip ? ip[i] : 0.0);
             cx.pose_prev[i] = is ? is[NP + i] : (iv ? iv[i] : 0.0);
             cx.vtarget[i] = 0.0;
-            cx.pid2prior[i] = -1;
+            cs.pid2prior[i] = -1;
         }
         if (tid < 3) cx.trans[tid] = is ? is[2 * NP + tid] : (it ? it[tid] : 0.0);
         if constexpr (XT) {
             const double* ish = chp->init_shape;
-            for (int e = tid; e < op.nshape; e += MOSHII_TPB) { cx.pose[NP + e] = is ? is[2 * NP + 5 + e] : (ish ? ish[e] : 0.0); cx.shp0[e] = 0.0; }
+            for (int e = tid; e < a_op.nshape; e += MOSHII_TPB) { cx.pose[NP + e] = is ? is[2 * NP + 5 + e] : (ish ? ish[e] : 0.0); cs.shp0[e] = 0.0; }
         }
         has_prev = is ? (is[2 * NP + 3] != 0.0) : (iv != nullptr);
         first = is ? (is[2 * NP + 4] != 0.0) : (chp->first != 0);
-    }
-    if (tid == 0) cx.scal[S_PRIOR_REF] = 0.0;
-    for (int i = tid; i < 8 * pr.npose + 16; i += MOSHII_TPB) cx.ell[i] = 0.0;
-    if (tid < md.K) cx.anc[tid] = md.anc[tid];
-    for (int i = tid; i < 3 * md.K; i += MOSHII_TPB) cx.Jl[i] = md.J[i];
-    __syncthreads();
-    for (int b = tid; b < op.nbody; b += MOSHII_TPB) cx.pid2prior[op.body[b]] = b;
-    __syncthreads();
+        if (tid == 0) cx.scal[S_PRIOR_REF] = 0.0;
+        for (int i = tid; i < 8 * a_pr.npose + 16; i += MOSHII_TPB) cs.ell[i] = 0.0;
+        if (tid < a_md.K) cs.anc[tid] = a_md.anc[tid];
+        for (int i = tid; i < 3 * a_md.K; i += MOSHII_TPB) cs.Jl[i] = a_md.J[i];
+        __syncthreads();
+        for (int b = tid; b < a_op.nbody; b += MOSHII_TPB) cs.pid2prior[a_op.body[b]] = b;
+        __syncthreads();
+    }
     int vc_key = 0, tab_key = 0;
     int rejoin_run = 0;
     int bi_next = 0;
@@ -2744,6 +3096,10 @@
     bool tail_cut = false;
     for (int t = 0; t <= F; ++t) {
         PROF_T(_tf);
+        const BodyArgs ka = body_args(reinterpret_cast<const KernelCtx*>(lds));
+        const auto& md = ka->md;
+        const auto& op = ka->op;
+        const auto& ly = ka->ly;
         if constexpr (!COOP && !XT) {
             if (chp->tail_done != nullptr && chp->tail_can_cut != 0 && t < F && F - t > chp->tail_left) {
                 if (tid == 0) cx.scal[S_ABORT] = (double)__hip_atomic_load(chp->tail_done, __ATOMIC_RELAXED, __HIP_MEMORY_SCOPE_AGENT);
@@ -2769,59 +3125,8 @@
             if (chp->baton != nullptr || chp->nb > 0 || chp->rejoin_tol > 0.0) {
                 bool halt = false;
                 if (lead) {
-                    const int S = 2 * NP + 5;
-                    if (rejoin_run >= 2 && t < F) {
-                        if (tid == 0 && chp->frames_done) *chp->frames_done = t;
-                        halt = true;
-                    }
-                    if (!halt && bi_next < chp->nb && t == chp->bnd[bi_next] - chp->bnd_off) {
-                        double* s1 = chp->run_final + (size_t)bi_next * S;
-                        for (int i = tid; i < NP; i += MOSHII_TPB) { s1[i] = cx.pose[i]; s1[NP + i] = cx.pose_prev[i]; }
-                        if (tid < 3) s1[2 * NP + tid] = cx.trans[tid];
-                        if (tid == 3) s1[2 * NP + 3] = has_prev ? 1.0 : 0.0;
-                        if (tid == 4) s1[2 * NP + 4] = first ? 1.0 : 0.0;
-                        if (chp->baton != nullptr) {
-                            if (tid == 0) {
-                                int* st = chp->baton + 2 * (chp->chunk0 + 1 + bi_next);
-                                double go = 1.0;
-                                if (__hip_atomic_load(st, __ATOMIC_ACQUIRE, __HIP_MEMORY_SCOPE_AGENT) == 1) {
-                                    __hip_atomic_store(st + 1, 1, __ATOMIC_RELEASE, __HIP_MEMORY_SCOPE_AGENT);
-                                    int spins = 0;
-                                    while (__hip_atomic_load(st, __ATOMIC_ACQUIRE, __HIP_MEMORY_SCOPE_AGENT) != 2) {
-                                        __builtin_amdgcn_s_sleep(64);
-                                        if (++spins > 20000) { go = 0.0; break; }
-                                    }
-                                }
-                                __builtin_amdgcn_fence(__ATOMIC_ACQUIRE, "agent");
-                                cx.scal[S_BATON] = go;
-                            }
-                            __syncthreads();
-                            if (cx.scal[S_BATON] == 0.0) { if (tid == 0 && chp->frames_done) *chp->frames_done = t; halt = true; }
-                            __syncthreads();
-                        }
-                        if (!halt) {
-                            double* s2 = chp->run_entry + (size_t)(bi_next + 1) * S;
-                            for (int i = tid; i < NP; i += MOSHII_TPB) { s2[i] = cx.pose[i]; s2[NP + i] = cx.pose_prev[i]; }
-                            if (tid < 3) s2[2 * NP + tid] = cx.trans[tid];
-                            if (tid == 3) s2[2 * NP + 3] = has_prev ? 1.0 : 0.0;
-                            if (tid == 4) s2[2 * NP + 4] = first ? 1.0 : 0.0;
-                            ++bi_next;
-                        }
-                    }
-                    if (!halt && chp->baton != nullptr && t < F) {
-                        if (tid == 0) cx.scal[S_ABORT] = (double)__hip_atomic_load(&chp->baton[2 * chp->chunk0 + 1], __ATOMIC_RELAXED, __HIP_MEMORY_SCOPE_AGENT);
-                        __syncthreads();
-                        if (cx.scal[S_ABORT] != 0.0) {
-                            if (tid == 0) {
-                                chp->run_entry[(size_t)bi_next * S + 2 * NP + 3] = MOSHII_MARK_ENTRY_SPOILED;
-                                int* mark = chp->abort_at + chp->chunk0 + bi_next;
-                                if (*mark < chp->bnd_off + t) *mark = chp->bnd_off + t;
-                                if (chp->frames_done) *chp->frames_done = -t - 1;
-                            }
-                            halt = true;
-                        }
-                        __syncthreads();
-                    }
+                    const int v = __builtin_amdgcn_readfirstlane(coop_lead_verdict_fn(chp, t, rejoin_run, bi_next, (has_prev ? 1 : 0) | (first ? 2 : 0)));
+                    halt = (v & 1) != 0; bi_next = v >> 1;
                 }
                 const unsigned seq = coop_begin(cx);
                 const double mine[1] = {halt ? 1.0 : 0.0};
@@ -2840,160 +3145,22 @@
             if (tid == 4) so[2 * NP + 4] = first ? 1.0 : 0.0;
             if constexpr (XT) for (int e = tid; e < op.nshape; e += MOSHII_TPB) so[2 * NP + 5 + e] = cx.pose[NP + e];
         }
-        if (!COOP && chp->fuse_flags != nullptr) {
-            const int S = 2 * NP + 5 + (XT ? op.nshape : 0);
-            if (t == skip && chp->entry_state != nullptr) {
-                __syncthreads();
-                if (tid == 0) { __threadfence(); __hip_atomic_store(&chp->fuse_flags[3 * chp->fuse_c], 1, __ATOMIC_RELEASE, __HIP_MEMORY_SCOPE_AGENT); }
-            }
-            if (chp->fuse_F == 0 && t == F) {
-                __syncthreads();
-                if (tid == 0) {
-                    __threadfence();
-                    __hip_atomic_store(&chp->fuse_flags[3 * chp->fuse_c + 1], 1, __ATOMIC_RELEASE, __HIP_MEMORY_SCOPE_AGENT);
-                    __hip_atomic_store(&chp->fuse_flags[3 * chp->fuse_c + 2], 1, __ATOMIC_RELEASE, __HIP_MEMORY_SCOPE_AGENT);
-                }
-            }
-            if (chp->fuse_F > 0 && t == chp->fuse_F) {
-                double* sf = chp->run_final - S;
-                for (int i = tid; i < NP; i += MOSHII_TPB) { sf[i] = cx.pose[i]; sf[NP + i] = cx.pose_prev[i]; }
-                if (tid < 3) sf[2 * NP + tid] = cx.trans[tid];
-                if (tid == 3) sf[2 * NP + 3] = has_prev ? 1.0 : 0.0;
-                if (tid == 4) sf[2 * NP + 4] = first ? 1.0 : 0.0;
-                if constexpr (XT) for (int e = tid; e < op.nshape; e += MOSHII_TPB) sf[2 * NP + 5 + e] = cx.pose[NP + e];
-                __syncthreads();
-                if (tid == 0) { __threadfence(); __hip_atomic_store(&chp->fuse_flags[3 * chp->fuse_c + 1], 1, __ATOMIC_RELEASE, __HIP_MEMORY_SCOPE_AGENT); }
-                bool carry = false;
-                auto state_dev = [&](const double* en) {
-                    double dv = 0.0, nn = 0.0;
-                    for (int i = tid; i < NP; i += MOSHII_TPB) { dv = fmax(dv, fmax(fabs(cx.pose[i] - en[i]), fabs(cx.pose_prev[i] - en[NP + i]))); nn += en[i] + en[NP + i]; }
-                    if (tid < 3) dv = fmax(dv, fabs(cx.trans[tid] - en[2 * NP + tid]));
-                    if (tid == 3 && (has_prev ? 1.0 : 0.0) != en[2 * NP + 3]) dv = MOSHII_HANDOFF_MISMATCH;
-                    if (tid == 4 && (first ? 1.0 : 0.0) != en[2 * NP + 4]) dv = MOSHII_HANDOFF_MISMATCH;
-                    if constexpr (XT) for (int e = tid; e < op.nshape; e += MOSHII_TPB) dv = fmax(dv, fabs(cx.pose[NP + e] - en[2 * NP + 5 + e]));
-                    if (!(nn == nn)) dv = MOSHII_HANDOFF_MISMATCH;
-                    return block_max(dv, cx.red);
-                };
-                auto wait_flag = [&](int* fl, int patience) {
-                    if (tid == 0) {
-                        double go = 1.0;
-                        int spins = 0;
-                        while (__hip_atomic_load(fl, __ATOMIC_ACQUIRE, __HIP_MEMORY_SCOPE_AGENT) != 1) {
-                            __builtin_amdgcn_s_sleep(64);
-                            if (++spins > patience) { go = 0.0; break; }
-                        }
-                        __builtin_amdgcn_fence(__ATOMIC_ACQUIRE, "agent");
-                        cx.scal[S_BATON] = go;
-                    }
-                    __syncthreads();
-                    const bool ok_ = cx.scal[S_BATON] != 0.0;
-                    __syncthreads();
-                    return ok_;
-                };
-                if (chp->fuse_has_next && wait_flag(chp->fuse_flags + 3 * (chp->fuse_c + 1), 2000)) {
-                    const double dv = state_dev(chp->run_entry);
-                    carry = !(dv <= chp->fuse_tol);
-                    if (carry && dv > 1e-6 && chp->fuse_has_prev && wait_flag(chp->fuse_flags + 3 * (chp->fuse_c - 1) + 1, 150)) {
-                        const double* lf = chp->run_final - 2 * S;
-                        const double* oe = chp->run_entry - S;
-                        double dl = 0.0;
-                        for (int i = tid; i < 2 * NP + 3; i += MOSHII_TPB) dl = fmax(dl, fabs(lf[i] - oe[i]));
-                        dl = block_max(dl, cx.red);
-                        if (!(dl <= 1e-6)) carry = false;
-                    }
-                }
-                if (carry && tid == 0) __hip_atomic_store(&chp->baton[2 * chp->chunk0], 1, __ATOMIC_RELEASE, __HIP_MEMORY_SCOPE_AGENT);
-                __syncthreads();
-                if (tid == 0) { __threadfence(); __hip_atomic_store(&chp->fuse_flags[3 * chp->fuse_c + 2], 1, __ATOMIC_RELEASE, __HIP_MEMORY_SCOPE_AGENT); }
-                if (!carry) { if (tid == 0 && chp->frames_done) *chp->frames_done = t; break; }
-                if (tid == 0) {
-                    int* fl = chp->fuse_flags + 3 * (chp->fuse_c + 1) + 1;
-                    double go = 1.0;
-                    int spins = 0;
-                    while (__hip_atomic_load(fl, __ATOMIC_ACQUIRE, __HIP_MEMORY_SCOPE_AGENT) != 1 ||
-                           __hip_atomic_load(fl + 1, __ATOMIC_ACQUIRE, __HIP_MEMORY_SCOPE_AGENT) != 1) {
-                        if (__hip_atomic_load(&chp->baton[2 * chp->chunk0 + 1], __ATOMIC_RELAXED, __HIP_MEMORY_SCOPE_AGENT) != 0) { go = 0.0; break; }
-                        __builtin_amdgcn_s_sleep(64);
-                        if (++spins > 20000) { go = 0.0; break; }
-                    }
-                    __builtin_amdgcn_fence(__ATOMIC_ACQUIRE, "agent");
-                    if (go != 0.0 && chp->fuse_count != nullptr) atomicAdd(chp->fuse_count, 1);
-                    cx.scal[S_BATON] = go;
-                }
-                __syncthreads();
-                if (cx.scal[S_BATON] == 0.0) { if (tid == 0 && chp->frames_done) *chp->frames_done = t; break; }
-                double* s2 = chp->run_entry;
-                for (int i = tid; i < NP; i += MOSHII_TPB) { s2[i] = cx.pose[i]; s2[NP + i] = cx.pose_prev[i]; }
-                if (tid < 3) s2[2 * NP + tid] = cx.trans[tid];
-                if (tid == 3) s2[2 * NP + 3] = has_prev ? 1.0 : 0.0;
-                if (tid == 4) s2[2 * NP + 4] = first ? 1.0 : 0.0;
-                if constexpr (XT) for (int e = tid; e < op.nshape; e += MOSHII_TPB) s2[2 * NP + 5 + e] = cx.pose[NP + e];
-                fuse_on = true;
+        if constexpr (!COOP) {
+            if (chp->fuse_flags != nullptr && (t == skip || t == chp->fuse_F || (t == F && chp->fuse_F == 0))) {
+                const int v = __builtin_amdgcn_readfirstlane(carry_on_fn<XT>(chp, t, (has_prev ? 1 : 0) | (first ? 2 : 0)));
+                if (v == 1) break;
+                if (v == 2) fuse_on = true;
             }
         }
         const bool sweeping = chp->fuse_F == 0 || fuse_on;
-        if (!COOP && bi_next < chp->nb && t == chp->bnd[bi_next] - chp->bnd_off) {
-            const int S = 2 * NP + 5 + (XT ? op.nshape : 0);
-            double* s1 = chp->run_final + (size_t)bi_next * S;
-            for (int i = tid; i < NP; i += MOSHII_TPB) { s1[i] = cx.pose[i]; s1[NP + i] = cx.pose_prev[i]; }
-            if (tid < 3) s1[2 * NP + tid] = cx.trans[tid];
-            if (tid == 3) s1[2 * NP + 3] = has_prev ? 1.0 : 0.0;
-            if (tid == 4) s1[2 * NP + 4] = first ? 1.0 : 0.0;
-            if constexpr (XT) for (int e = tid; e < op.nshape; e += MOSHII_TPB) s1[2 * NP + 5 + e] = cx.pose[NP + e];
-            if (chp->baton != nullptr) {
-                if (tid == 0) {
-                    int* st = chp->baton + 2 * (chp->chunk0 + 1 + bi_next);
-                    double go = 1.0;
-                    if (chp->fuse_flags != nullptr) {
-                        int* vd = chp->fuse_flags + 3 * (chp->chunk0 + bi_next) + 2;
-                        int spins = 0;
-                        while (__hip_atomic_load(vd, __ATOMIC_ACQUIRE, __HIP_MEMORY_SCOPE_AGENT) != 1) {
-                            __builtin_amdgcn_s_sleep(64);
-                            if (++spins > 20000) { go = 0.0; break; }
-                        }
-                    }
-                    if (go != 0.0 && __hip_atomic_load(st, __ATOMIC_ACQUIRE, __HIP_MEMORY_SCOPE_AGENT) == 1) {
-                        __hip_atomic_store(st + 1, 1, __ATOMIC_RELEASE, __HIP_MEMORY_SCOPE_AGENT);
-                        int spins = 0;
-                        while (__hip_atomic_load(st, __ATOMIC_ACQUIRE, __HIP_MEMORY_SCOPE_AGENT) != 2) {
-                            __builtin_amdgcn_s_sleep(64);
-                            if (++spins > 20000) { go = 0.0; break; }
-                        }
-                    }
-                    if (go != 0.0 && chp->fuse_flags != nullptr) {
-                        int* od = chp->fuse_flags + 3 * (chp->chunk0 + 1 + bi_next) + 1;
-                        int spins = 0;
-                        while (__hip_atomic_load(od, __ATOMIC_ACQUIRE, __HIP_MEMORY_SCOPE_AGENT) != 1) {
-                            __builtin_amdgcn_s_sleep(64);
-                            if (++spins > 20000) { go = 0.0; break; }
-                        }
-                    }
-                    __builtin_amdgcn_fence(__ATOMIC_ACQUIRE, "agent");
-                    cx.scal[S_BATON] = go;
-                }
-                __syncthreads();
-                if (cx.scal[S_BATON] == 0.0) { if (tid == 0 && chp->frames_done) *chp->frames_done = t; break; }
-            }
-            double* s2 = chp->run_entry + (size_t)(bi_next + 1) * S;
-            for (int i = tid; i < NP; i += MOSHII_TPB) { s2[i] = cx.pose[i]; s2[NP + i] = cx.pose_prev[i]; }
-            if (tid < 3) s2[2 * NP + tid] = cx.trans[tid];
-            if (tid == 3) s2[2 * NP + 3] = has_prev ? 1.0 : 0.0;
-            if (tid == 4) s2[2 * NP + 4] = first ? 1.0 : 0.0;
-            if constexpr (XT) for (int e = tid; e < op.nshape; e += MOSHII_TPB) s2[2 * NP + 5 + e] = cx.pose[NP + e];
-            ++bi_next;
-        }
-        if (!COOP && chp->baton != nullptr && sweeping && t < F) {
-            if (tid == 0) cx.scal[S_ABORT] = (double)__hip_atomic_load(&chp->baton[2 * chp->chunk0 + 1], __ATOMIC_RELAXED, __HIP_MEMORY_SCOPE_AGENT);
-            __syncthreads();
-            if (cx.scal[S_ABORT] != 0.0) {
-                if (tid == 0) {
-                    const int S = 2 * NP + 5 + (XT ? op.nshape : 0);
-                    chp->run_entry[(size_t)bi_next * S + 2 * NP + 3] = MOSHII_MARK_ENTRY_SPOILED;
-                    int* mark = chp->abort_at + chp->chunk0 + bi_next;
-                    if (*mark < chp->bnd_off + t) *mark = chp->bnd_off + t;
-                    if (chp->frames_done) *chp->frames_done = -t - 1;
-                }
-                break;
+        if constexpr (!COOP) {
+            const int stf = (has_prev ? 1 : 0) | (first ? 2 : 0);
+            if (bi_next < chp->nb && t == chp->bnd[bi_next] - chp->bnd_off) {
+                if (__builtin_amdgcn_readfirstlane(chunk_boundary_fn<XT>(chp, t, bi_next, stf)) == 0) break;
+                ++bi_next;
+            }
+            if (chp->baton != nullptr && sweeping && t < F) {
+                if (__builtin_amdgcn_readfirstlane(territory_request_fn<XT>(chp, t, bi_next)) != 0) break;
             }
         }
         if (t == F) break;
@@ -3040,7 +3207,8 @@
         if constexpr (XT) {
             fp.wt_poseF = op.wt_poseF * anneal;
             fp.has_stay = (!first && op.wt_shape_stay != 0.0) ? 1 : 0;
-            for (int e = tid; e < op.nshape; e += MOSHII_TPB) cx.shp0[e] = cx.pose[NP + e];
+            double* shp0 = lds + ly.o_shp0;
+            for (int e = tid; e < op.nshape; e += MOSHII_TPB) shp0[e] = cx.pose[NP + e];
         }
         fp.has_velo = has_prev ? 1 : 0;
         if (has_prev)
@@ -3067,7 +3235,7 @@
             }
             const int terms = fp.use_fingers | (fp.use_face << 1) | (fp.use_shape << 2);
             const bool reuse = at_pose && prev_wt_pose == fp.wt_pose && prev_terms == terms;
-            fin = run_phase<NBLK, XT, COOP>(cx, ly, md, at, pr, op, fp, visrow, step2 ? op.step2 : op.step1, step2 ? op.n2 : op.n1,
+            fin = run_phase<NBLK, XT, COOP>(cx, fp, visrow, step2, step2 ? op.n2 : op.n1,
                                   (XT && step2) ? op.nshape : 0, XT ? chp->qscratch + (COOP ? (size_t)co.rank * chp->coop.qstride : 0) : nullptr,
                                   round ? op.e3_first : op.e3, kind == 0, kind == 5, reuse, carried, at_pose, fwd_set,
                                   (kind >= 4 && !same_sets) ? 2 : 1, vc_key, tab_key, n_iter, n_fev, fail, co);
diff --git a/moshpp_amd/csrc/moshii_api.hip b/moshpp_amd/csrc/moshii_api.hip
--- a/moshpp_amd/csrc/moshii_api.hip
+++ b/moshpp_amd/csrc/moshii_api.hip
@@ -1281,6 +1281,10 @@
     int rc;
     if ((rc = check_opts(m, prior, o, &d))) return rc;
     if ((rc = choose_layout(m, d, Mmax, Nvmax, NWmax, n_workgroups, coop_g, cfg))) return rc;
+#ifdef MOSHII_EMULATION
+    if (getenv("MOSHII_TEST_BREAK_LAYOUT")) { cfg->ly.o_dgn += 2; cfg->ly.o_ddl += 2; cfg->ly.o_y += 2; cfg->ly.o_red += 2; cfg->ly.o_scal += 2; }
+#endif
+    if (const char* why = chain_layout_fault(cfg->ly, cfg->nblk)) return fail(MOSHII_ERR_UNSUPPORTED, std::string("internal error: ") + why);
     return upload_ids(m, prior, o, stream, extra_bytes, cfg, ctl_off);
 }
 
diff --git a/moshpp_amd/csrc/moshii_dev.h b/moshpp_amd/csrc/moshii_dev.h
--- a/moshpp_amd/csrc/moshii_dev.h
+++ b/moshpp_amd/csrc/moshii_dev.h
@@ -157,6 +157,15 @@
     int i_visidx, i_colpid, i_colprior, i_pid2prior, i_jointslot, i_kfree, i_colq, i_ksum, i_kconst, i_total;
     int t_Jh, t_Jrow, t_Lm, t_Trot, t_xjs, t_rest, t_tjs;
 };
+inline const char* chain_layout_fault(const ChainLayout& ly, int nblk) {
+    const int LDJ = 16 * nblk;
+    if (nblk <= 0 || ly.LDJ != LDJ) return "chain layout: LDJ is not 16 register blocks";
+    if (ly.o_dsd - ly.o_g != LDJ || ly.o_dgn - ly.o_g != 2 * LDJ || ly.o_ddl - ly.o_g != 3 * LDJ || ly.o_y - ly.o_g != 4 * LDJ)
+        return "chain layout: the control vectors g, dsd, dgn, ddl, y are not LDJ doubles apart";
+    if (ly.o_red - ly.o_g != 5 * LDJ || ly.o_scal - ly.o_red != 16) return "chain layout: red / scal do not follow the control vectors";
+    if (ly.i_colprior - ly.i_colpid != LDJ) return "chain layout: colprior is not LDJ ints behind colpid";
+    return nullptr;
+}
 
 struct KernelCtx {
     ChainLayout ly;
```

After: 67350 (median of 6 runs). 1.7% higher.
